# jonicho/simd-radix-sort

Measured on AMD Instinct MI355X. Metric: Gkeys/s and achieved HBM GB/s (% of roofline), 1e9 uint64 key+uint64 payload, higher is better.
Workload: dtype uint64; 1 GPU; c1: 1e9 uint64 keys + one uint64 payload column, uniform random; keys_per_gpu=1000000000, total_keys=1000000000, record_bytes=16, parallelism=1 GPU

## Files before the change

### include/srs_c_api.h

```cpp
#ifndef SRS_C_API_H_
#define SRS_C_API_H_

#include <stdint.h>

#ifdef __cplusplus
extern "C" {
#endif

typedef enum srs_key_kind {
  SRS_KEY_U8 = 0,
  SRS_KEY_I8 = 1,
  SRS_KEY_U16 = 2,
  SRS_KEY_I16 = 3,
  SRS_KEY_U32 = 4,
  SRS_KEY_I32 = 5,
  SRS_KEY_U64 = 6,
  SRS_KEY_I64 = 7,
  SRS_KEY_F32 = 8,
  SRS_KEY_F64 = 9
} srs_key_kind;

typedef enum srs_status {
  SRS_OK = 0,
  SRS_ERR_INVALID_ARG = -1,
// ... 62 lines not shown
                             const void* const* payloads, const uint32_t* payload_sizes,
                             void* keys_out, void* const* payloads_out,
                             int64_t* indices_out, void* stream);
int64_t srs_topk_rows_max_k(void);


int srs_key_histogram_device(int64_t num, int key_kind, int up, const void* keys,
                             int bits, uint64_t* hist, void* stream);

int srs_partition_device(int64_t num, int key_kind, int up, const void* keys,
                         int32_t num_payloads, const void* const* payloads,
                         const uint32_t* payload_sizes, int bits,
                         const int32_t* part_of_bucket, int32_t num_parts,
                         void* keys_out, void* const* payloads_out,
                         int64_t* part_counts, void* stream);

#define SRS_SHARD_ID_BYTES 128
typedef struct srs_shard_comm_s* srs_shard_comm;
int srs_shard_unique_id(void* id);
int srs_shard_comm_init(int32_t world, int32_t rank, const void* id, srs_shard_comm* comm);
int srs_shard_comm_init_all(int32_t num_devices, const int32_t* devices, srs_shard_comm* comms);
int srs_shard_comm_destroy(srs_shard_comm comm);

int srs_shard_comm_init_staged(int32_t world, srs_shard_comm* comms);

int srs_shard_set_options(srs_shard_comm comm, int32_t rounds, int32_t chunks);

int srs_shard_set_message_options(srs_shard_comm comm, int32_t self_messages,
                                  int64_t max_message_bytes);

int srs_shard_sort_device(srs_shard_comm comm, int64_t num, int key_kind, int up,
                          const void* keys, int32_t num_payloads, const void* const* payloads,
                          const uint32_t* payload_sizes, void** keys_out, void** payloads_out,
                          int64_t* num_out, void* stream);

int srs_shard_sort_multi(int32_t num_devices, const srs_shard_comm* comms, const int64_t* nums,
                         int key_kind, int up, const void* const* keys, int32_t num_payloads,
                         const void* const* payloads, const uint32_t* payload_sizes,
                         void** keys_out, void** payloads_out, int64_t* nums_out);

int srs_shard_last_report(srs_shard_comm comm, char* buf, int64_t cap);

int srs_shard_debug_inject(srs_shard_comm comm, int32_t point);

int srs_debug_shard_plan(int32_t world, int32_t rank, int32_t chunks, int32_t rounds,
                         int32_t key_bits, int32_t self_messages, const uint64_t* chunk_hists,
                         int64_t num, char* json, int64_t cap);


int srs_set_host_devices(int32_t num_devices, const int32_t* devices);


int srs_alloc_device(uint64_t bytes, void** ptr);
int srs_free_device(void* ptr);


int srs_fill_synthetic_device(int64_t num, int key_kind, uint64_t seed,
                              uint64_t first_index, void* keys,
                              int32_t num_payloads, void* const* payloads,
                              const uint32_t* payload_sizes, void* stream);


const char* srs_last_error(void);

const char* srs_version(void);

int srs_set_kernel_timing(int enable);
int srs_reset_kernel_stats(void);
int srs_kernel_stats(const char* name, int64_t* launches, double* total_ms,
                     double* elements);

int srs_debug_set_stamp_buffer(void* device_acc);

int srs_debug_set_lookback(void* status, void* err);

int srs_debug_set_super_scan(int64_t min_groups);

int srs_debug_last_fallbacks(int64_t* counts);

int srs_debug_last_local_counts(int64_t* counts);

int srs_debug_last_local_classes(int64_t* counts);

int srs_debug_alloc(uint64_t bytes, int mode, void** ptr);
int srs_debug_free(void* ptr);
int srs_debug_workspace(void** tmp, uint64_t* tmp_bytes, void** tmp2, uint64_t* tmp2_bytes);
int srs_debug_probe_write(void* ptr, uint64_t bytes, float* ms);

int srs_debug_plan_table(const uint32_t* hist, int64_t num, int key_bits, int32_t* mode,
                         int32_t* groups, double* overflow, double* overflow_other,
                         int32_t* table, int32_t* rbits);

int srs_release_workspace(void);

int srs_debug_set_topk_candidates(int64_t max_candidates);

int srs_debug_last_topk(int64_t* info);

int srs_debug_set_topk_rows_route(int route);

int srs_debug_last_topk_rows(int64_t* info);

#ifdef __cplusplus
}
#endif

#endif
```

### simd-radix-sort_amd/csrc/srs_api.hip

```cpp
#include <hip/hip_runtime.h>
#include <stdint.h>
#include <string.h>

#include <algorithm>
#include <atomic>
#include <chrono>
#include <cstring>
#include <cstdio>
#include <cstdlib>
#include <map>
#include <memory>
#include <mutex>
#include <queue>
#include <string>
#include <thread>
#include <vector>

#include "../../include/srs_c_api.h"
#include "srs_common.h"
#include "srs_kernels.h"

namespace srs {
namespace {

// ... 358 lines not shown
  auto it = g_pub_allocs.upper_bound(const_cast<void*>(p));
  if (it == g_pub_allocs.begin()) return false;
  --it;
  const char* a = (const char*)it->first;
  return (const char*)p >= a && (const char*)p + bytes <= a + it->second;
}

thread_local bool t_defer = false;
thread_local std::vector<std::pair<void*, int>> t_deferred;

hipError_t ws_free(void* p, int mode) {
  if (!p) return hipSuccess;
  if (t_defer) {
    t_deferred.push_back({p, mode});
    return hipSuccess;
  }
  return big_free(p, mode);
}

int ensure(DevBuf& b, size_t bytes, int mode = ALLOC_MALLOC, bool placed = false) {
  if (b.bytes >= bytes && b.p) return SRS_OK;
  if (b.p) {
    HIP_TRY(ws_free(b.p, b.mode));
    b.p = nullptr;
    b.bytes = 0;
  }
  size_t want = std::max<size_t>(bytes, 256);
  if (placed) HIP_TRY(placed_alloc(&b.p, want, mode));
  else HIP_TRY(big_alloc(&b.p, want, mode));
  b.bytes = want;
  b.mode = mode;
  return SRS_OK;
}

int ensure_keep(DevBuf& b, size_t bytes, size_t live_bytes, hipStream_t st) {
  if (b.bytes >= bytes && b.p) return SRS_OK;
  DevBuf nb;
  size_t want = std::max<size_t>(bytes, b.bytes * 2);
  HIP_TRY(hipMalloc(&nb.p, want));
  nb.bytes = want;
  if (b.p && live_bytes) HIP_TRY(hipMemcpyAsync(nb.p, b.p, live_bytes, hipMemcpyDeviceToDevice, st));
  if (b.p) {
    HIP_TRY(hipStreamSynchronize(st));
    HIP_TRY(ws_free(b.p, ALLOC_MALLOC));
  }
  b = nb;
  return SRS_OK;
}

inline void cpu_relax() {
#if defined(__x86_64__) || defined(__i386__)
  __builtin_ia32_pause();
#else
  std::this_thread::yield();
#endif
}

int sync_poll(hipStream_t st) {
  const auto t0 = std::chrono::steady_clock::now();
  for (;;) {
    const hipError_t q = hipStreamQuery(st);
    if (q == hipSuccess) return SRS_OK;
    if (q != hipErrorNotReady) HIP_TRY(q);
    const auto dt = std::chrono::steady_clock::now() - t0;
    if (dt > std::chrono::milliseconds(20)) break;
    if (dt < std::chrono::microseconds(200)) cpu_relax();
    else std::this_thread::yield();
  }
  HIP_TRY(hipStreamSynchronize(st));
  return SRS_OK;
}

struct Workspace {
  DevBuf tmp;
  DevBuf tmp2;
  DevBuf stage;
  DevBuf desc;
  DevBuf big[2], local, local2, copy, fallback, fallback2, redo, redo2;
  DevBuf plan, tcount, gcount, tbase, gbase, var, sbase;
  DevBuf tile_seg, group_seg, hist, offs, gsum, gofs, scan_tmp, totals, ctr;
  DevBuf shist, lut, lut_rbits;
  DevBuf prun, ptile, btot, bnt, btile, nt_over, gtile, gorder;
  int64_t gorder_cap = 0;
  DevBuf mid;
  DevBuf midbar;
  DevBuf sel, selhist, selcnt, seldesc;
  unsigned long long* h_sel = nullptr;
  int64_t topk_info[3] = {0, 0, 0};
  DevBuf rowspass;
  int64_t topk_rows_info[4] = {0, 0, 0, 0};
  bool rows_pass_pending = false;
  hipStream_t side = nullptr;
  hipEvent_t ev_fork = nullptr, ev_join = nullptr;
  ListCounters* h_ctr = nullptr;
  uint64_t* h_totals = nullptr;
  MidFlag* h_mid = nullptr;
  unsigned long long mid_seq = 0;
  hipEvent_t idle = nullptr;
  bool idle_pending = false;
  std::map<hipStream_t, DevBuf> small_taken;
  bool last_small = false;
  hipStream_t last_small_stream = nullptr;
  std::mutex mu;
  ~Workspace() {
    if (idle) {
      (void)hipEventSynchronize(idle);
      (void)hipEventDestroy(idle);
    }
    DevBuf* bufs[] = {&tmp, &tmp2, &stage, &desc, &big[0], &big[1], &local, &local2, &fallback,
                      &fallback2, &redo, &redo2, &shist, &lut, &lut_rbits, &copy, &plan, &tcount,
                      &gcount, &tbase, &gbase, &var, &sbase, &tile_seg, &group_seg, &hist, &offs,
                      &gsum, &gofs, &scan_tmp, &totals, &ctr, &prun, &ptile, &btot, &bnt, &btile,
                      &nt_over, &gtile, &gorder, &mid, &midbar, &sel, &selhist, &selcnt, &seldesc,
                      &rowspass};
    for (DevBuf* b : bufs) free_buf(*b);
    for (auto& t : small_taken) free_buf(t.second);
    if (h_sel) (void)hipHostFree(h_sel);
    if (h_ctr) (void)hipHostFree(h_ctr);
    if (h_totals) (void)hipHostFree(h_totals);
    if (h_mid) (void)hipHostFree(h_mid);
    if (side) (void)hipStreamDestroy(side);
    if (ev_fork) (void)hipEventDestroy(ev_fork);
    if (ev_join) (void)hipEventDestroy(ev_join);
    (void)hipGetLastError();
  }
};

std::mutex g_wmu;
std::map<int, std::shared_ptr<Workspace>>& g_ws = *new std::map<int, std::shared_ptr<Workspace>>;

struct WsLock {
  std::shared_ptr<Workspace> ref;
  std::unique_lock<std::mutex> lk;
};

int get_ws_locked(std::shared_ptr<Workspace>* out) {
  int dev = 0;
  HIP_TRY(hipGetDevice(&dev));
  auto it = g_ws.find(dev);
  if (it != g_ws.end()) {
    *out = it->second;
    return SRS_OK;
  }
  auto w = std::make_shared<Workspace>();
  HIP_TRY(hipHostMalloc((void**)&w->h_ctr, sizeof(ListCounters), hipHostMallocDefault));
  HIP_TRY(hipHostMalloc((void**)&w->h_totals, 4 * sizeof(uint64_t), hipHostMallocDefault));
  HIP_TRY(hipHostMalloc((void**)&w->h_mid, sizeof(MidFlag), hipHostMallocCoherent));
  memset(w->h_mid, 0, sizeof(MidFlag));
  g_ws[dev] = w;
  *out = w;
  return SRS_OK;
}

int acquire_ws(Workspace** out, WsLock* lk) {
  std::shared_ptr<Workspace> w;
  {
    std::lock_guard<std::mutex> g(g_wmu);
    SRS_TRY(get_ws_locked(&w));
  }
  lk->lk = std::unique_lock<std::mutex>(w->mu);
  lk->ref = std::move(w);
  *out = lk->ref.get();
  return SRS_OK;
}

size_t align_up(size_t x, size_t a) { return (x + a - 1) / a * a; }
// ... 447 lines not shown
      ok = (int)cl.size() <= kMaxRanges && cl.back().b1 - cl.back().b0 < kClusterSpan;
    }
    if (ok) {
      *clusters = cl;
      return SRS_OK;
    }
  }
  if (top9max * 512 <= (uint64_t)kBalancedSkew * total) {
    *spread = true;
    return SRS_OK;
  }
  if (R.aos) return SRS_OK;
  TablePlan P;
  plan_table(h, n, d.key_bits, &P);
  if (trace_levels() && P.mode)
    fprintf(stderr, "[srs] digit table mode %d: %d groups, predicted overflow %.0f keys (other "
            "table %.0f)\n", P.mode, P.groups, P.over, P.over_other);
  if (P.mode == 0) return SRS_OK;
  std::vector<int32_t>& rbits = P.rbits;
  if (P.mode == 3) {
    SRS_TRY(ensure(W->lut, 512 * sizeof(int32_t)));
    SRS_TRY(ensure(W->lut_rbits, kGroups * sizeof(int32_t)));
    HIP_TRY(hipMemcpyAsync(W->lut.p, P.tab3.data(), 512 * 4, hipMemcpyHostToDevice, st));
    HIP_TRY(hipMemcpyAsync(W->lut_rbits.p, rbits.data(), rbits.size() * 4, hipMemcpyHostToDevice,
                           st));
    HIP_TRY(hipStreamSynchronize(st));
    *lut_entries = 1024;
    *lut_mode = 3;
    *use = true;
    return SRS_OK;
  }
  const std::vector<int32_t>& lut = P.lut16;
  std::vector<uint16_t> t2(4096);
  for (int B = 0; B < 4096; B++) {
    bool same = true;
    for (int j = 1; j < 16; j++) same &= lut[B * 16 + j] == lut[B * 16];
    if (same) {
      t2[B] = (uint16_t)lut[B * 16];
    } else {
      const int idx = (int)(t2.size() - 4096) / 16;
      t2[B] = (uint16_t)(0x8000 | idx);
      for (int j = 0; j < 16; j++) t2.push_back((uint16_t)lut[B * 16 + j]);
    }
  }
  if ((int)t2.size() > kLdsLutEntries) return fail(SRS_ERR_INTERNAL, "digit table too large");
  *lut_entries = (int)t2.size();
  SRS_TRY(ensure(W->lut, align_up(t2.size() * sizeof(uint16_t), 16)));
  SRS_TRY(ensure(W->lut_rbits, kGroups * sizeof(int32_t)));
  HIP_TRY(hipMemcpyAsync(W->lut.p, t2.data(), t2.size() * 2, hipMemcpyHostToDevice, st));
  HIP_TRY(hipMemcpyAsync(W->lut_rbits.p, rbits.data(), rbits.size() * 4, hipMemcpyHostToDevice,
                         st));
  HIP_TRY(hipStreamSynchronize(st));
  *use = true;
  return SRS_OK;
}

int pair_tiles_mode(const SortDesc& d, int ks, bool aos_slices) {
  const char* e = getenv("SRS_PAIR_TILES");
  const int mode = e && *e ? atoi(e) : 2;
  if (mode == 0 || d.canon_zero || (ks != 4 && ks != 8)) return 0;
  const bool shape = d.cols[0].width == (uint32_t)ks &&
                     (d.pair ? ks == 4 && d.ncols == 3 : d.ncols <= 2);
  if (!shape) return 0;
  if (mode == 3) return 1 | 2;
  if (mode == 1) return 1;
  return aos_slices ? (1 | 4) : ks == 4 ? (1 | 2) : 1;
}

struct LevelState {
  int64_t nbig, n_local, n_local2, n_copy;
  int cur;
  int ncols;
  int tmp2;
  int64_t known_len = -1;
  int pair_tiles = 0;
  int level = 0;
};

struct LevelMode {
  int mode = 0;
  const GTile* gt = nullptr;
  const int32_t* nt_over = nullptr;
  const int32_t* torder = nullptr;
  int key_bits = 0;
  bool home = false;
};

int run_level(Workspace* W, int ks, const SortDesc* d_desc, LevelState& S, int force_bits,
              int lut, hipStream_t st, const int32_t* lut_rbits = nullptr,
              const LevelMode& M = LevelMode()) {
  const int64_t nbig = S.nbig;
  ListCounters* d_ctr = (ListCounters*)W->ctr.p;
  uint64_t* d_totals = (uint64_t*)W->totals.p;
  SRS_TRY(ensure(W->plan, nbig * sizeof(SegPlan)));
  SRS_TRY(ensure(W->tcount, nbig * 8));
  SRS_TRY(ensure(W->gcount, nbig * 8));
  SRS_TRY(ensure(W->tbase, nbig * 8));
  SRS_TRY(ensure(W->gbase, nbig * 8));
  SRS_TRY(ensure(W->var, nbig * 16));
  SRS_TRY(ensure(W->sbase, (size_t)nbig * kMaxBins * 8));
  SRS_TRY(ensure(W->scan_tmp, scan_temp_elems(nbig) * 8));
  SegPlan* plan = (SegPlan*)W->plan.p;
  unsigned long long* var = (unsigned long long*)W->var.p;
  const bool small_plan = nbig <= kPlanSmallMax;
  if (small_plan) {
    TimedScope ts("plan", (double)nbig, st);
    launch_plan_small((Seg*)W->big[S.cur].p, nbig, plan, (int64_t*)W->tbase.p,
                      (int64_t*)W->gbase.p, var, d_totals, &d_ctr->n_big, force_bits,
                      S.tmp2 | (M.home ? 2 : 0), st, M.nt_over);
  } else {
    TimedScope ts("plan", (double)nbig, st);
    HIP_TRY(hipMemsetAsync(d_totals + 3, 0, sizeof(uint64_t), st));
    launch_plan((Seg*)W->big[S.cur].p, nbig, plan, (int64_t*)W->tcount.p,
                (int64_t*)W->gcount.p, var, d_totals + 3, force_bits, S.tmp2 | (M.home ? 2 : 0),
                st, M.nt_over);
    launch_excl_scan((uint64_t*)W->tcount.p, (uint64_t*)W->tbase.p, nbig,
                     (uint64_t*)W->scan_tmp.p, d_totals + 0, st);
    launch_excl_scan((uint64_t*)W->gcount.p, (uint64_t*)W->gbase.p, nbig,
                     (uint64_t*)W->scan_tmp.p, d_totals + 1, st);
    launch_plan_bases(plan, nbig, (int64_t*)W->tbase.p, (int64_t*)W->gbase.p, st);
  }
  int64_t ntiles, ngroups;
  uint64_t level_keys;
  if (nbig == 1 && S.known_len >= 0) {
    level_keys = (uint64_t)S.known_len;
    ntiles = (S.known_len + kTile - 1) / kTile;
    ngroups = (ntiles + kScanGroup - 1) / kScanGroup;
  } else {
    HIP_TRY(hipMemcpyAsync(W->h_totals, d_totals, 4 * sizeof(uint64_t),
                           hipMemcpyDeviceToHost, st));
    SRS_TRY(sync_poll(st));
    ntiles = (int64_t)W->h_totals[0];
    ngroups = (int64_t)W->h_totals[1];
    level_keys = W->h_totals[3];
  }
  S.known_len = -1;
  const int lv = ++S.level;
  const double level_elems = (double)level_keys;
  note_elems("count", level_elems, lv);
  note_elems("scatter", level_elems, lv);

  SRS_TRY(ensure(W->tile_seg, ntiles * 4));
  SRS_TRY(ensure(W->group_seg, ngroups * 4));
  SRS_TRY(ensure(W->hist, (size_t)ntiles * kMaxBins * 2));
  const bool offs32 = level_keys < (1ull << 32);
  SRS_TRY(ensure(W->offs, (size_t)ntiles * kMaxBins * (offs32 ? 4 : 8)));
  const int64_t grows = ngroups + super_rows(ngroups);
  SRS_TRY(ensure(W->gsum, (size_t)grows * kMaxBins * 4));
  SRS_TRY(ensure(W->gofs, (size_t)grows * kMaxBins * 8));
  int32_t* tile_seg = (int32_t*)W->tile_seg.p;
  int32_t* group_seg = (int32_t*)W->group_seg.p;
  launch_seg_map2((int64_t*)W->tbase.p, ntiles, tile_seg, (int64_t*)W->gbase.p, ngroups,
                  group_seg, nbig, st);
  {
    TimedScope ts("count", (double)0, st, lv);
    launch_count(ks, d_desc, plan, tile_seg, ntiles, (uint16_t*)W->hist.p, var, var + nbig, lut, st,
                 M.gt, M.torder);
  }
  const size_t worst = (size_t)nbig * kMaxBins;
  const int nxt = S.cur ^ 1;
  SRS_TRY(ensure(W->big[nxt], worst * sizeof(Seg)));
  SRS_TRY(ensure_keep(W->local, (S.n_local + worst) * sizeof(Seg), S.n_local * sizeof(Seg), st));
  SRS_TRY(ensure_keep(W->local2, (S.n_local2 + worst) * sizeof(Seg), S.n_local2 * sizeof(Seg), st));
  SRS_TRY(ensure_keep(W->copy, (S.n_copy + worst) * sizeof(Seg), S.n_copy * sizeof(Seg), st));
  if (!small_plan)
    HIP_TRY(hipMemsetAsync(&d_ctr->n_big, 0, sizeof(unsigned long long), st));
  {
    TimedScope ts("scan", (double)ntiles, st);
    launch_offsets(plan, nbig, group_seg, ngroups, (uint16_t*)W->hist.p,
                   (uint32_t*)W->gsum.p, (uint64_t*)W->gofs.p, (uint64_t*)W->sbase.p,
                   offs32 ? nullptr : (uint64_t*)W->offs.p, offs32 ? (uint32_t*)W->offs.p : nullptr,
                   var, (Seg*)W->big[nxt].p, (Seg*)W->local.p,
                   (Seg*)W->local2.p, (Seg*)W->copy.p, d_ctr, lut_rbits, st, M.mode,
                   (uint32_t*)W->prun.p);
  }
  if (g_lb_status)
    HIP_TRY(hipMemsetAsync(g_lb_status, 0, (size_t)ntiles * kMaxBins * 4, st));
  {
    TimedScope ts("scatter", (double)0, st, lv);
    const bool pairs = (S.pair_tiles & 1) && (lut == 0 || ((S.pair_tiles & 2) && lut == 2)) &&
                       !((S.pair_tiles & 4) && lv == 1);
    if (pairs)
      launch_scatter_pairs(ks, d_desc, plan, tile_seg, (uint64_t*)W->offs.p,
                           offs32 ? (const uint32_t*)W->offs.p : nullptr, ntiles, lut, st, M.gt);
    else
      launch_scatter(ks, d_desc, plan, tile_seg, (uint64_t*)W->offs.p,
                     offs32 ? (const uint32_t*)W->offs.p : nullptr, ntiles, lut, S.ncols, st,
                     M.gt);
  }
  if (M.mode == 1) {
    const int nb = 1 << std::abs(force_bits);
    const int rbits = lut ? M.key_bits : M.key_bits - std::abs(force_bits);
    launch_stripe_tables((const uint32_t*)W->prun.p, nbig, nb, (uint32_t*)W->ptile.p,
                         (uint64_t*)W->btot.p, (uint32_t*)W->bnt.p, rbits, BUF_TMP,
                         (Seg*)W->big[nxt].p, (int32_t*)W->nt_over.p, (uint32_t*)W->btile.p,
                         d_ctr, (const uint64_t*)W->sbase.p, plan, (GTile*)W->gtile.p,
                         lut_rbits, st, (int32_t*)W->gorder.p, W->gorder_cap);
  }
  HIP_TRY(hipMemcpyAsync(W->h_ctr, d_ctr, sizeof(ListCounters), hipMemcpyDeviceToHost, st));
  SRS_TRY(sync_poll(st));
  S.nbig = (int64_t)W->h_ctr->n_big;
  S.n_local = (int64_t)W->h_ctr->n_local;
  S.n_local2 = (int64_t)W->h_ctr->n_local2;
  S.n_copy = (int64_t)W->h_ctr->n_copy;
  S.cur = nxt;
  if (trace_levels()) {
    fprintf(stderr, "[srs] level: %lld segs, %.0f keys, %lld tiles%s -> big %lld, local %lld, "
            "local2 %lld, copy %lld\n", (long long)nbig, level_elems, (long long)ntiles,
            lut ? " (lut)" : "", (long long)S.nbig, (long long)S.n_local,
            (long long)S.n_local2, (long long)S.n_copy);
    if (S.nbig > 0) {
      std::vector<Seg> b(S.nbig);
      HIP_TRY(hipMemcpy(b.data(), W->big[nxt].p, S.nbig * sizeof(Seg), hipMemcpyDeviceToHost));
      int64_t sum = 0, mx = 0, under16k = 0;
      for (const Seg& s : b) {
        sum += s.len;
        mx = std::max<int64_t>(mx, s.len);
        under16k += s.len <= 16384;
      }
      fprintf(stderr, "[srs]   big: %lld keys, max %lld, <= 16K keys: %lld segs; first rbits %d\n",
              (long long)sum, (long long)mx, (long long)under16k, b[0].rbits);
    }
  }
  return SRS_OK;
}

void set_columns(const Request& R, SortDesc& d, char* tmp, char* tmp2, bool aos_cols,
                 size_t slice_bytes, const size_t* tmp_off, bool inplace, bool pair = false) {
  const int ks = key_size_of(R.kind);
  if (R.aos) {
    const uint32_t E = R.elem_size;
    char* in = (char*)R.in_cols[0];
    char* out = (char*)R.out_cols[0];
    const uint32_t slice = E < 8 ? E : 8;
    int nc = 0;
    for (uint32_t off = 0; off < E; off += slice, nc++) {
      if (aos_cols)
        d.cols[nc] = Col{{in + off, out + off, tmp + nc * slice_bytes, tmp2 + nc * slice_bytes},
                         slice, {E, E, 8, 8}};
      else
        d.cols[nc] = Col{{in + off, out + off, tmp ? tmp + off : nullptr, nullptr}, slice,
                         {E, E, E, E}};
    }
    d.ncols = nc;
    d.key = d.cols[0];
    d.key.width = (uint32_t)ks;
  } else {
    for (int c = 0; c < R.ncols; c++) {
      const uint32_t w = R.widths[c];
      d.cols[c] = Col{{(char*)R.in_cols[c], (char*)R.out_cols[c], tmp ? tmp + tmp_off[c] : nullptr,
                       tmp2 ? tmp2 + tmp_off[c] : nullptr}, w, {w, w, w, w}};
    }
    if (pair) {
      for (int c = 1; c <= 2; c++) {
        const size_t off = tmp_off[1] + 4 * (c - 1);
        d.cols[c].base[BUF_TMP] = tmp + off;
        d.cols[c].base[BUF_TMP2] = tmp2 + off;
        d.cols[c].stride[BUF_TMP] = d.cols[c].stride[BUF_TMP2] = 8;
      }
      d.pair = 1;
    }
    d.key = d.cols[0];
    d.ncols = R.ncols;
  }
  if (inplace)
    for (int c = 0; c < d.ncols; c++) d.cols[c].base[BUF_IN] = d.cols[c].base[BUF_OUT];
}

bool is_inplace(const Request& R) {
  bool inplace = true;
  for (int c = 0; c < R.ncols; c++) inplace &= (R.in_cols[c] == R.out_cols[c]);
  return inplace;
}

int taken_slot(Workspace* W, hipStream_t st, DevBuf** out) {
  if (W->small_taken.size() >= 64 && !W->small_taken.count(st)) {
    HIP_TRY(hipDeviceSynchronize());
    for (auto& t : W->small_taken) free_buf(t.second);
    W->small_taken.clear();
    W->last_small = false;
  }
  DevBuf& taken = W->small_taken[st];
  SRS_TRY(ensure(taken, 2 * sizeof(int64_t)));
  *out = &taken;
  return SRS_OK;
}

int run_small(Workspace* W, const Request& R, hipStream_t st) {
  const int ks = key_size_of(R.kind);
  const int64_t n = R.num;
  const bool inplace = is_inplace(R);
  SortDesc d;
  memset(&d, 0, sizeof d);
  key_masks(R.kind, R.up, d);
  const bool is_float = R.kind == SRS_KEY_F32 || R.kind == SRS_KEY_F64;
  d.canon_zero = (is_float && n <= R.thresh) ? 1 : 0;
  d.leaf_skip = leaf_skip_of(R);
  const int ksl = ks | (d.canon_zero ? SRS_KS_CANON : 0);
  set_columns(R, d, nullptr, nullptr, false, 0, nullptr, inplace);
  d.stamp_acc = g_stamp_acc;
  const Seg g{0, n, d.key_bits, inplace ? BUF_OUT : BUF_IN};
  DevBuf* tk = nullptr;
  SRS_TRY(taken_slot(W, st, &tk));
  DevBuf& taken = *tk;
  W->last_small = true;
  W->last_small_stream = st;
  note_elems("local", (double)n);
  {
    TimedScope ts("local", (double)0, st);
    launch_small_sort(ksl, d, g, (int64_t*)taken.p, st);
  }
  HIP_TRY(hipGetLastError());
  return SRS_OK;
}

bool direct_layout_ok(const SortDesc& d, int pm, int ks) {
  const Col& k = d.cols[0];
  const int bufs[] = {BUF_IN, BUF_OUT, BUF_TMP, BUF_TMP2};
  if (pm == 0) {
    if (d.ncols != 2 || d.pair || d.cols[1].width != 8 || k.width != (uint32_t)ks) return false;
    for (int b : {BUF_IN, BUF_OUT, BUF_TMP, BUF_TMP2}) {
      if (b == BUF_TMP2 && !d.tmp2) continue;
      if (k.stride[b] != k.width || d.cols[1].stride[b] != 8) return false;
    }
    return true;
  }
  if (pm == 1) {
    const Col& p = d.cols[1];
    if (d.ncols != 2 || !d.tmp2 || ks != 8 || k.width != 8 || p.width != 8) return false;
    for (int b : {BUF_IN, BUF_OUT})
      if (k.stride[b] != 16 || p.stride[b] != 16 || p.base[b] != k.base[b] + 8) return false;
    for (int b : {BUF_TMP, BUF_TMP2})
      if (k.stride[b] != 8 || p.stride[b] != 8) return false;
    return true;
  }
  if (pm == 2) {
    const Col& a = d.cols[1];
    const Col& c = d.cols[2];
    if (d.ncols != 3 || !d.pair || a.width != 4 || c.width != 4 || k.width != (uint32_t)ks)
      return false;
    for (int b : bufs)
      if (k.stride[b] != k.width) return false;
    for (int b : {BUF_IN, BUF_OUT})
      if (a.stride[b] != 4 || c.stride[b] != 4) return false;
    for (int b : {BUF_TMP, BUF_TMP2})
      if (a.stride[b] != 8 || c.stride[b] != 8 || c.base[b] != a.base[b] + 4) return false;
    return true;
  }
  return false;
}

constexpr int64_t kStripeMinN = int64_t(1) << 25;

bool stripes_enabled() {
  static const bool on = [] {
    const char* e = getenv("SRS_NO_STRIPES");
    return !(e && *e && *e != '0');
  }();
  return on;
}

int plan_range_level(Workspace* W, const Request& R, const std::vector<KeyCluster>& cl,
                     SortDesc& d, hipStream_t st, bool* use, bool* final_lvl, bool* one_value) {
  *use = *final_lvl = *one_value = false;
  const int ks = key_size_of(R.kind);
  const int kb = 8 * ks;
  const int K = (int)cl.size();
  uint64_t hi[kMaxRanges] = {~0ull, ~0ull, ~0ull, ~0ull};
  for (int k = 0; k + 1 < K; k++) {
    const uint64_t mid_bin = ((uint64_t)cl[k].b1 + (uint64_t)cl[k + 1].b0 + 1) / 2;
    hi[k] = (mid_bin << (kb - 16)) - 1;
  }
  SRS_TRY(ensure(W->totals, 2 * kMaxRanges * sizeof(uint64_t)));
  unsigned long long* mm = (unsigned long long*)W->totals.p;
  uint64_t init[2 * kMaxRanges];
  for (int c = 0; c < kMaxRanges; c++) {
    init[2 * c] = ~0ull;
    init[2 * c + 1] = 0;
  }
  std::vector<uint64_t> got(2 * kMaxRanges);
  HIP_TRY(hipMemcpyAsync(mm, init, sizeof init, hipMemcpyHostToDevice, st));
  launch_key_minmax(R.in_cols[0], ks, ks, R.num, d.mpos, d.mneg, hi, mm, st);
  HIP_TRY(hipMemcpyAsync(got.data(), mm, sizeof init, hipMemcpyDeviceToHost, st));
  SRS_TRY(sync_poll(st));
  struct Rg {
    uint64_t mn, mx, cnt, hi;
  };
  std::vector<Rg> rg;
  for (int c = 0; c < K; c++) {
    if (got[2 * c] > got[2 * c + 1]) continue;
    rg.push_back(Rg{got[2 * c], got[2 * c + 1], std::max<uint64_t>(cl[c].cnt, 1), hi[c]});
  }
  if (rg.empty()) return SRS_OK;
  if (rg.size() == 1 && rg[0].mn == rg[0].mx) {
    *one_value = true;
    return SRS_OK;
  }
  const int R_ = (int)rg.size();
  auto shr = [](uint64_t x, int s) { return s >= 64 ? 0 : x >> s; };
  auto span = [&](int s) {
    uint64_t t = 0;
    for (const Rg& r : rg) t += shr(r.mx, s) - shr(r.mn, s) + 1;
    return t;
  };
  int s = 0;
  while (s < kb && span(s) > (uint64_t)kMaxBins) s++;
  uint32_t used = 0;
  for (int c = 0; c < kMaxRanges; c++) {
    d.rng_hi[c] = ~0ull;
    d.rng_adj[c] = 0;
  }
  std::vector<int> base(R_);
  for (int c = 0; c < R_; c++) {
    d.rng_hi[c] = c + 1 < R_ ? rg[c].hi : ~0ull;
    base[c] = (int)used;
    d.rng_adj[c] = used - (uint32_t)shr(rg[c].mn, s);
    used += (uint32_t)(shr(rg[c].mx, s) - shr(rg[c].mn, s) + 1);
  }
  std::vector<int32_t> rbits(kMaxBins, s);
  SRS_TRY(ensure(W->lut_rbits, kMaxBins * sizeof(int32_t)));
  HIP_TRY(hipMemcpyAsync(W->lut_rbits.p, rbits.data(), kMaxBins * sizeof(int32_t),
                         hipMemcpyHostToDevice, st));
  HIP_TRY(hipStreamSynchronize(st));
  d.digit_lut = nullptr;
  d.lut_mode = 2;
  d.lut_bits = kMaxDigitBits;
  d.lut_shift = s;
  d.lut_entries = 0;
  *use = true;
  *final_lvl = s == 0;
  if (trace_levels())
    for (int c = 0; c < R_; c++)
      fprintf(stderr, "[srs] range %d: keys [%llx, %llx] -> buckets from %d, shift %d\n", c,
              (unsigned long long)rg[c].mn, (unsigned long long)rg[c].mx, base[c], s);
  return SRS_OK;
}

int copy_through(const Request& R, hipStream_t st);

constexpr int64_t kHomeTmp2MinN = int64_t(1) << 24;

bool home_tmp2_enabled() {
  static const bool on = [] {
    const char* e = getenv("SRS_HOME_TMP2");
    return !(e && *e == '0');
  }();
  return on;
}

bool partition_pairs_enabled() {
  static const bool on = [] {
    const char* e = getenv("SRS_PARTITION_PAIRS");
    return !(e && *e == '0');
  }();
  return on;
}

constexpr int64_t kLocalForkMaxN = int64_t(1) << 24;
bool local_fork_enabled() {
  static const bool on = [] {
    const char* e = getenv("SRS_LOCAL_FORK");
    return !(e && *e == '0');
  }();
  return on;
}

bool mid_enabled() {
  static const bool on = [] {
    const char* e = getenv("SRS_MID");
    return !(e && *e == '0');
  }();
  return on;
}

int64_t mid_level_max_n() {
  static const int64_t v = [] {
    const char* e = getenv("SRS_MID_LEVEL_MAX");
    const int64_t x = e && *e ? (int64_t)atof(e) : kMidLevelMaxKeys;
    return std::min<int64_t>(x, kMidLevelMaxKeys);
  }();
  return v;
}

int wait_mid_flag(const MidFlag* f, unsigned long long seq, hipStream_t st) {
  auto seen = [&] { return __atomic_load_n(&f->seq, __ATOMIC_ACQUIRE) == seq; };
  const auto t0 = std::chrono::steady_clock::now();
  while (!seen()) {
    if (std::chrono::steady_clock::now() - t0 > std::chrono::milliseconds(5)) {
      HIP_TRY(hipStreamSynchronize(st));
      if (!seen()) return fail(SRS_ERR_INTERNAL, "mid-size launch: no answer from the kernel");
      break;
    }
    cpu_relax();
  }
  return SRS_OK;
}

int run_sort(Workspace* W, const Request& R, hipStream_t st) {
  if (R.nsegs == 0 && R.num <= kLocalCap) return run_small(W, R, st);
  {
    const char* e = getenv("SRS_XCD_ROT");
    set_xcd_rotation(e && *e ? atoi(e) : 0);
  }
  W->last_small = false;
  const int ks = key_size_of(R.kind);
  const int64_t n = R.num;
  const bool inplace = is_inplace(R);

  SortDesc d;
  memset(&d, 0, sizeof d);
  key_masks(R.kind, R.up, d);
  const bool is_float = R.kind == SRS_KEY_F32 || R.kind == SRS_KEY_F64;
  d.canon_zero = (is_float && n <= R.thresh) ? 1 : 0;
  d.leaf_skip = leaf_skip_of(R);
  const int ksl = ks | (d.canon_zero ? SRS_KS_CANON : 0);
  const bool mid = R.nsegs == 0 && n > kLocalCap && n <= kMidMaxKeys && mid_enabled();
  const bool mid1 = R.nsegs == 0 && n > kMidMaxKeys && n <= mid_level_max_n() && mid_enabled();

  const bool aos_cols = R.aos && R.elem_size >= 16 && n > kLocalCap && R.nsegs == 0 && !mid;
  const bool pair_cols = !R.aos && R.ncols == 3 && R.widths[1] == 4 && R.widths[2] == 4 &&
                         n > kLocalCap && R.nsegs == 0 && !mid && !mid1;
  bool home_tmp2 = false;
  if (!R.aos && !pair_cols && n >= kHomeTmp2MinN && R.nsegs == 0 && !mid && !mid1 &&
      home_tmp2_enabled()) {
    for (int c = 0; c < R.ncols && !home_tmp2; c++)
      home_tmp2 = !placed_memory(R.out_cols[c], (size_t)n * R.widths[c]);
  }
  size_t tmp_bytes = 0, slice_bytes = 0;
  std::vector<size_t> tmp_off;
  if (R.aos) {
    tmp_off.push_back(0);
    slice_bytes = align_up((size_t)n * 8, 256);
    tmp_bytes = aos_cols ? slice_bytes * (R.elem_size / 8) : align_up((size_t)n * R.elem_size, 256);
  } else {
    for (int c = 0; c < R.ncols; c++) {
      tmp_off.push_back(tmp_bytes);
      tmp_bytes += align_up((size_t)n * R.widths[c], 256);
    }
  }
  SRS_TRY(ensure(W->tmp, tmp_bytes, ws_alloc_mode(), true));
  char* tmp = (char*)W->tmp.p;
  char* tmp2 = nullptr;
  if (home_tmp2 && ensure(W->tmp2, tmp_bytes, ws_alloc_mode(), true) != SRS_OK) {
    home_tmp2 = false;
    (void)hipGetLastError();
  }
  if (aos_cols || pair_cols || home_tmp2) {
    SRS_TRY(ensure(W->tmp2, tmp_bytes, ws_alloc_mode(), true));
    tmp2 = (char*)W->tmp2.p;
    d.tmp2 = 1;
  }

  set_columns(R, d, tmp, tmp2, aos_cols, slice_bytes, tmp_off.data(), inplace, pair_cols);

  d.stamp_acc = g_stamp_acc;
  d.lb_status = g_lb_status;
  d.lb_err = g_lb_err;
  bool balanced = false, spread = false, ranges = false, ranges_final = false;
  int lut_entries = 0, lut_mode = 1;
  std::vector<KeyCluster> clusters;
  SRS_TRY(plan_balanced_level(W, R, d, &balanced, &lut_entries, &lut_mode, st, &spread,
                              &clusters));
  if (!clusters.empty()) {
    bool one_value = false;
    SRS_TRY(plan_range_level(W, R, clusters, d, st, &ranges, &ranges_final, &one_value));
    if (one_value) return copy_through(R, st);
    balanced = ranges;
  }
  if (balanced && !ranges) {
    d.digit_lut = (const int32_t*)W->lut.p;
    d.lut_shift = d.key_bits - (lut_mode == 3 ? 9 : 16);
    d.lut_bits = lut_mode == 3 ? 9 : 16;
    d.lut_mode = lut_mode;
    d.lut_entries = lut_entries;
  }
  SRS_TRY(ensure(W->desc, sizeof(SortDesc)));
  SortDesc* d_desc = (SortDesc*)W->desc.p;

  const int home = inplace ? BUF_OUT : BUF_IN;
  SRS_TRY(ensure(W->big[0], 1024 * sizeof(Seg)));
  SRS_TRY(ensure(W->big[1], 1024 * sizeof(Seg)));
  SRS_TRY(ensure(W->local, 1024 * sizeof(Seg)));
  SRS_TRY(ensure(W->local2, 1024 * sizeof(Seg)));
  SRS_TRY(ensure(W->copy, 1024 * sizeof(Seg)));
  SRS_TRY(ensure(W->ctr, sizeof(ListCounters)));
  SRS_TRY(ensure(W->totals, 4 * sizeof(uint64_t)));
  ListCounters* d_ctr = (ListCounters*)W->ctr.p;
// ... 86 lines not shown
          W->last_small_stream = st;
          return SRS_OK;
        }
        launch_set_desc(d, d_desc, st);
        W->h_ctr->local_elems = 0;
        started = true;
      }
    }
    if (mid1) {
      const int64_t T = (n + kTile - 1) / kTile;
      const int64_t part_bytes = mid_level_part_bytes();
      SRS_TRY(ensure(W->mid, part_bytes + T * kMaxBins * sizeof(uint32_t)));
      if (!W->midbar.p) {
        SRS_TRY(ensure(W->midbar, mid_bar_words() * sizeof(unsigned long long)));
        HIP_TRY(hipMemsetAsync(W->midbar.p, 0, mid_bar_words() * sizeof(unsigned long long), st));
      }
      auto barrier_failed = [&] { return __atomic_load_n(&W->h_mid->err, __ATOMIC_ACQUIRE) != 0; };
      if (barrier_failed())
        return fail(SRS_ERR_INTERNAL, "mid-size launch: a grid barrier timed out");
      hipError_t e;
      const unsigned long long seq = ++W->mid_seq;
      {
        note_elems("mid_level", (double)n);
        TimedScope ts("mid_level", (double)0, st);
        e = launch_mid_level(ksl, d, n, home, (unsigned long long*)W->mid.p,
                             (uint32_t*)((char*)W->mid.p + part_bytes), d_ctr, (Seg*)W->big[0].p,
                             (Seg*)W->local.p, (Seg*)W->local2.p, (Seg*)W->copy.p, d_desc,
                             W->h_mid, seq, (unsigned long long*)W->midbar.p, st);
      }
      if (e != hipSuccess) {
        (void)hipGetLastError();
        if (trace_levels())
          fprintf(stderr, "[srs] mid-level launch refused (%s): general path\n", hipGetErrorString(e));
      } else {
        SRS_TRY(wait_mid_flag(W->h_mid, seq, st));
        if (barrier_failed())
          return fail(SRS_ERR_INTERNAL, "mid-size launch: a grid barrier timed out");
        n_big = (int64_t)__atomic_load_n(&W->h_mid->n_big, __ATOMIC_ACQUIRE);
        n_local = (int64_t)__atomic_load_n(&W->h_mid->n_local, __ATOMIC_ACQUIRE);
        n_local2 = (int64_t)__atomic_load_n(&W->h_mid->n_local2, __ATOMIC_ACQUIRE);
        n_copy = (int64_t)__atomic_load_n(&W->h_mid->n_copy, __ATOMIC_ACQUIRE);
        W->h_ctr->local_elems = __atomic_load_n(&W->h_mid->local_elems, __ATOMIC_ACQUIRE);
        if (trace_levels())
          fprintf(stderr, "[srs] mid-level: big %lld, local %lld, local2 %lld, copy %lld\n",
                  (long long)n_big, (long long)n_local, (long long)n_local2, (long long)n_copy);
        if (n_big + n_local + n_local2 + n_copy == 0) return SRS_OK;
        started = true;
      }
    }
    if (!started) {
      Seg seg0{0, n, d.key_bits, home};
      const bool to_local = n <= kLocalCap;
      launch_start(d, d_desc, seg0, to_local ? 1 : 0, (Seg*)W->big[0].p, (Seg*)W->local.p,
                   (Seg*)W->local2.p, d_ctr, st);
      n_big = to_local ? 0 : 1;
      n_local = (to_local && n <= kLocalCapSmall) ? 1 : 0;
      n_local2 = (to_local && n > kLocalCapSmall) ? 1 : 0;
      W->h_ctr->local_elems = to_local ? (uint64_t)n : 0;
    } else {
      mid_continued = true;
    }
  }
  LevelState S{n_big, n_local, n_local2, n_copy, 0, d.ncols, d.tmp2};
  S.pair_tiles = pair_tiles_mode(d, ks, aos_cols);
  if (R.nsegs == 0 && n_big == 1 && !mid_continued) S.known_len = n;
  if (one_seg_len > 0) S.known_len = one_seg_len;
  int level = 0;
  const int b1 = balanced ? kMaxDigitBits : choose_bits(n, d.key_bits);
  const int64_t stripe_len = (int64_t)kStripeKeysPerBucket << b1;
  const bool stripes = R.nsegs == 0 && !d.canon_zero && (ks == 4 || ks == 8) &&
                       (balanced || spread) && !ranges_final &&
                       n >= kStripeMinN && n < (int64_t(1) << 32) && n >= 2 * stripe_len &&
                       stripes_enabled();
  if (stripes) {
    const int64_t K = (n + stripe_len - 1) / stripe_len;
    std::vector<Seg> hs(K);
    for (int64_t k = 0; k < K; k++)
      hs[k] = Seg{k * stripe_len, std::min(stripe_len, n - k * stripe_len), d.key_bits, home};
    SRS_TRY(ensure(W->big[0], K * sizeof(Seg)));
    HIP_TRY(hipMemcpyAsync(W->big[0].p, hs.data(), K * sizeof(Seg), hipMemcpyHostToDevice, st));
    const int nb = 1 << b1;
    const size_t pieces = (size_t)K * kMaxBins;
    SRS_TRY(ensure(W->prun, pieces * 4));
    SRS_TRY(ensure(W->ptile, pieces * 4));
    SRS_TRY(ensure(W->btot, kMaxBins * 8));
    SRS_TRY(ensure(W->bnt, kMaxBins * 4));
    SRS_TRY(ensure(W->btile, kMaxBins * 4));
    SRS_TRY(ensure(W->nt_over, kMaxBins * 4));
    SRS_TRY(ensure(W->gtile, ((n + kTile - 1) / kTile + (size_t)K * nb) * sizeof(GTile)));
    W->gorder_cap = (n + kTile - 1) / kTile + (int64_t)K * nb;
    SRS_TRY(ensure(W->gorder, (W->gorder_cap + K) * sizeof(int32_t)));
    HIP_TRY(hipStreamSynchronize(st));
    S.nbig = K;
    S.known_len = -1;
    LevelMode m1;
    m1.mode = 1;
    m1.key_bits = d.key_bits;
    ++level;
    if (balanced)
      SRS_TRY(run_level(W, ksl, d_desc, S, kMaxDigitBits, d.lut_mode >= 2 ? 2 : 1, st,
                        (const int32_t*)W->lut_rbits.p, m1));
    else
      SRS_TRY(run_level(W, ksl, d_desc, S, -b1, false, st, nullptr, m1));
    LevelMode m2;
    m2.mode = 2;
    m2.gt = (const GTile*)W->gtile.p;
    m2.nt_over = (const int32_t*)W->nt_over.p;
    m2.torder = (const int32_t*)W->gorder.p;
    ++level;
    if (S.nbig > 0) SRS_TRY(run_level(W, ksl, d_desc, S, 0, false, st, nullptr, m2));
  }
  if (balanced && !stripes && S.nbig > 0) {
    ++level;
    LevelMode m0;
    m0.home = ranges_final;
    SRS_TRY(run_level(W, ksl, d_desc, S, kMaxDigitBits, d.lut_mode >= 2 ? 2 : 1, st,
                      (const int32_t*)W->lut_rbits.p, m0));
  }
  while (S.nbig > 0) {
    if (++level > 80) return fail(SRS_ERR_INTERNAL, "level limit exceeded");
    SRS_TRY(run_level(W, ksl, d_desc, S, 0, false, st));
  }
  n_local = S.n_local;
  n_local2 = S.n_local2;
  n_copy = S.n_copy;

  if (n_local + n_local2 > 0) {
    note_elems("local", (double)W->h_ctr->local_elems);
    TimedScope ts("local", (double)0, st);
    SRS_TRY(ensure(W->fallback, (n_local + n_local2) * sizeof(Seg)));
    SRS_TRY(ensure(W->fallback2, (n_local + n_local2) * sizeof(Seg)));
    Seg* fb = (Seg*)W->fallback.p;
    Seg* fb1 = fb + n_local2;
    Seg* fb2 = (Seg*)W->fallback2.p;
    unsigned long long* nfb = &d_ctr->n_fallback;
    unsigned long long* nfb1 = &d_ctr->n_fallback1;
    unsigned long long* nfb2 = &d_ctr->n_fallback2;
    hipStream_t s2 = st;
    if (n_local > 0 && n_local2 > 0 && n <= kLocalForkMaxN && local_fork_enabled()) {
      if (!W->side) {
        HIP_TRY(hipStreamCreateWithFlags(&W->side, hipStreamNonBlocking));
        HIP_TRY(hipEventCreateWithFlags(&W->ev_fork, hipEventDisableTiming));
        HIP_TRY(hipEventCreateWithFlags(&W->ev_join, hipEventDisableTiming));
      }
      HIP_TRY(hipEventRecord(W->ev_fork, st));
      HIP_TRY(hipStreamWaitEvent(W->side, W->ev_fork, 0));
      s2 = W->side;
    }
    {
      TimedScope ts1("local_fast", 0, st);
      const bool rec16 = aos_cols && R.elem_size == 16;
      int pm = -1;
      if (!R.aos && R.ncols == 2 && R.widths[1] == 8 && !d.pair) pm = 0;
      else if (rec16 && ks == 8) pm = 1;
      else if (d.pair && ks == 4) pm = 2;
      if (pm >= 0 && !direct_layout_ok(d, pm, ks)) pm = -1;
      const bool direct_any = pm >= 0 && (ks == 4 || ks == 8) && !d.canon_zero &&
                              direct_local_enabled();
      const bool direct = direct_any && n_local >= direct_min_segs();
      const bool direct2 = direct_any && direct_local2_enabled() && n_local2 >= direct_min_segs();
      if (n_local2 > 0 && direct2) {
        SRS_TRY(ensure(W->redo2, n_local2 * sizeof(Seg)));
        launch_local_direct(ks, pm, d_desc, (Seg*)W->local2.p, n_local2, (Seg*)W->redo2.p,
                            &d_ctr->n_redo2, fb, nfb, s2, true);
        launch_local_list(ks, d_desc, (Seg*)W->redo2.p, &d_ctr->n_redo2,
                          (int)std::min<int64_t>(n_local2, 1024), fb, nfb, s2, true);
      } else if (n_local2 > 0) {
        launch_local(ksl, d_desc, (Seg*)W->local2.p, n_local2, 1, fb, nfb, s2, rec16);
      }
      if (n_local > 0 && direct) {
        SRS_TRY(ensure(W->redo, n_local * sizeof(Seg)));
        launch_local_direct(ks, pm, d_desc, (Seg*)W->local.p, n_local, (Seg*)W->redo.p,
                            &d_ctr->n_redo, fb1, nfb1, st);
        launch_local_list(ks, d_desc, (Seg*)W->redo.p, &d_ctr->n_redo,
                          (int)std::min<int64_t>(n_local, 2048), fb1, nfb1, st);
      } else if (n_local > 0) {
        launch_local(ksl, d_desc, (Seg*)W->local.p, n_local, 0, fb1, nfb1, st, rec16);
      }
    }
    {
// ... 1308 lines not shown
int srs_set_host_devices(int32_t num_devices, const int32_t* devices) {
  if (num_devices < 0 || num_devices > 512 || (num_devices > 0 && !devices))
    return fail(SRS_ERR_INVALID_ARG, "num_devices must be in [0, 512] with a device array");
  int ndev = 0;
  if (num_devices > 0 && (hipGetDeviceCount(&ndev) != hipSuccess || ndev == 0))
    return fail(SRS_ERR_NO_DEVICE, "no HIP device available");
  for (int i = 0; i < num_devices; i++)
    if (devices[i] < 0 || devices[i] >= ndev)
      return fail(SRS_ERR_INVALID_ARG, "no such device in the host device list");
  std::lock_guard<std::mutex> g(g_hdmu);
  g_host_devs.assign(devices, devices + num_devices);
  g_host_devs_set = true;
  return SRS_OK;
}

int srs_set_kernel_timing(int enable) {
  std::lock_guard<std::mutex> lk(g_tmu);
  g_timing = enable == 2 ? 2 : enable != 0;
  return SRS_OK;
}

int srs_reset_kernel_stats(void) {
  std::lock_guard<std::mutex> lk(g_tmu);
  drain_timing_locked();
  g_stats.clear();
  return SRS_OK;
}

int srs_kernel_stats(const char* name, int64_t* launches, double* total_ms, double* elements) {
  std::lock_guard<std::mutex> lk(g_tmu);
  drain_timing_locked();
  if (!name) return fail(SRS_ERR_INVALID_ARG, "name is NULL");
  auto it = g_stats.find(name);
  const KStat k = it == g_stats.end() ? KStat{} : it->second;
  if (launches) *launches = k.launches;
  if (total_ms) *total_ms = k.ms;
  if (elements) *elements = k.elems;
  return SRS_OK;
}

int srs_debug_set_stamp_buffer(void* device_acc) {
  g_stamp_acc = (unsigned long long*)device_acc;
  return SRS_OK;
}

int srs_debug_set_lookback(void* status, void* err) {
  g_lb_status = (uint32_t*)status;
  g_lb_err = (unsigned long long*)err;
  return SRS_OK;
}

int srs_debug_last_local_counts(int64_t* counts) {
  if (!counts) return fail(SRS_ERR_INVALID_ARG, "counts is NULL");
  Workspace* W = nullptr;
  WsLock lk;
  SRS_TRY(acquire_ws(&W, &lk));
  counts[0] = counts[1] = 0;
  if (W->last_small || !W->ctr.p) return SRS_OK;
  HIP_TRY(hipDeviceSynchronize());
  ListCounters c;
  HIP_TRY(hipMemcpy(&c, W->ctr.p, sizeof c, hipMemcpyDeviceToHost));
  counts[0] = (int64_t)(c.n_local + c.n_local2);
  counts[1] = (int64_t)(c.n_redo + c.n_redo2);
  return SRS_OK;
}

int srs_debug_last_local_classes(int64_t* counts) {
  if (!counts) return fail(SRS_ERR_INVALID_ARG, "counts is NULL");
  Workspace* W = nullptr;
  WsLock lk;
  SRS_TRY(acquire_ws(&W, &lk));
  counts[0] = counts[1] = counts[2] = counts[3] = 0;
  if (W->last_small || !W->ctr.p) return SRS_OK;
  HIP_TRY(hipDeviceSynchronize());
  ListCounters c;
  HIP_TRY(hipMemcpy(&c, W->ctr.p, sizeof c, hipMemcpyDeviceToHost));
  counts[0] = (int64_t)c.n_local;
  counts[1] = (int64_t)c.n_local2;
  counts[2] = (int64_t)c.n_redo;
  counts[3] = (int64_t)c.n_redo2;
  return SRS_OK;
}

int srs_debug_set_super_scan(int64_t min_groups) {
  set_super_scan_min_groups(min_groups);
  return SRS_OK;
}

int srs_debug_last_fallbacks(int64_t* counts) {
  if (!counts) return fail(SRS_ERR_INVALID_ARG, "counts is NULL");
  Workspace* W = nullptr;
  WsLock lk;
  SRS_TRY(acquire_ws(&W, &lk));
  counts[0] = counts[1] = 0;
  if (W->last_small) {
    HIP_TRY(hipDeviceSynchronize());
    HIP_TRY(hipMemcpy(counts, W->small_taken[W->last_small_stream].p, 2 * sizeof(int64_t),
                      hipMemcpyDeviceToHost));
    return SRS_OK;
  }
  if (!W->ctr.p) return SRS_OK;
  HIP_TRY(hipDeviceSynchronize());
  ListCounters c;
  HIP_TRY(hipMemcpy(&c, W->ctr.p, sizeof c, hipMemcpyDeviceToHost));
  counts[0] = (int64_t)(c.n_fallback + c.n_fallback1);
  counts[1] = (int64_t)c.n_fallback2;
  return SRS_OK;
}

int srs_debug_plan_table(const uint32_t* hist, int64_t num, int key_bits, int32_t* mode,
                         int32_t* groups, double* overflow, double* overflow_other,
                         int32_t* table, int32_t* rbits) {
  if (!hist || !mode || !table || !rbits || (key_bits != 32 && key_bits != 64) || num < 1)
    return fail(SRS_ERR_INVALID_ARG, "srs_debug_plan_table: arguments");
  std::vector<uint32_t> h(hist, hist + 65536);
  TablePlan P;
  plan_table(h, num, key_bits, &P);
  *mode = P.mode;
  if (groups) *groups = P.groups;
  if (overflow) *overflow = P.over;
  if (overflow_other) *overflow_other = P.over_other;
  if (P.mode == 1) memcpy(table, P.lut16.data(), 65536 * 4);
  if (P.mode == 3) memcpy(table, P.tab3.data(), 512 * 4);
  if (P.mode) memcpy(rbits, P.rbits.data(), kGroups * 4);
  return SRS_OK;
}

int srs_alloc_device(uint64_t bytes, void** ptr) {
  if (!ptr) return fail(SRS_ERR_INVALID_ARG, "srs_alloc_device: ptr is NULL");
  *ptr = nullptr;
  if (bytes == 0) return SRS_OK;
  HIP_TRY(placed_alloc(ptr, (size_t)bytes, ALLOC_MALLOC));
  std::lock_guard<std::mutex> g(g_pub_amu);
  g_pub_allocs[*ptr] = (size_t)bytes;
  return SRS_OK;
}

int srs_free_device(void* ptr) {
  if (!ptr) return SRS_OK;
  {
    std::lock_guard<std::mutex> g(g_pub_amu);
    auto it = g_pub_allocs.find(ptr);
    if (it == g_pub_allocs.end())
      return fail(SRS_ERR_INVALID_ARG, "srs_free_device: not from srs_alloc_device");
    g_pub_allocs.erase(it);
  }
  HIP_TRY(hipFree(ptr));
  return SRS_OK;
}

std::mutex g_dbg_amu;
std::map<void*, int> g_dbg_allocs;

int srs_debug_alloc(uint64_t bytes, int mode, void** ptr) {
  if (!ptr || mode < ALLOC_MALLOC || mode >= ALLOC_MODES || bytes == 0)
    return fail(SRS_ERR_INVALID_ARG, "srs_debug_alloc: ptr, mode 0..4 and bytes > 0");
  HIP_TRY(big_alloc(ptr, (size_t)bytes, mode));
  std::lock_guard<std::mutex> g(g_dbg_amu);
  g_dbg_allocs[*ptr] = mode;
  return SRS_OK;
}

int srs_debug_free(void* ptr) {
  int mode = 0;
  {
    std::lock_guard<std::mutex> g(g_dbg_amu);
// ... 91 lines not shown
```

### simd-radix-sort_amd/csrc/srs_common.h

```cpp
#pragma once

#include <hip/hip_runtime.h>
#include <stdint.h>

namespace srs {

enum BufId : int32_t { BUF_IN = 0, BUF_OUT = 1, BUF_TMP = 2, BUF_TMP2 = 3 };
constexpr int kNumBufs = 4;

struct Col {
  char* base[kNumBufs];
  uint32_t width;
  uint32_t stride[kNumBufs];
};

#define SRS_MAX_COLS 65

struct SortDesc {
  Col key;
  Col cols[SRS_MAX_COLS];
  int32_t ncols;
  int32_t key_bits;
  int32_t canon_zero;
  int32_t tmp2;
  int32_t pair;
  int32_t leaf_skip;
  uint64_t mpos, mneg, signbit, negzero;
  const int32_t* digit_lut;
  int32_t lut_shift;
  int32_t lut_bits;
  int32_t lut_mode;
  int32_t lut_entries;
  uint64_t rng_hi[4];
  uint32_t rng_adj[4];
  unsigned long long* stamp_acc;
  uint32_t* lb_status;
  unsigned long long* lb_err;
};

struct Seg {
  int64_t start;
  int64_t len;
  int32_t rbits;
  int32_t buf;
};

struct SegPlan {
  int64_t start;
  int64_t len;
  int64_t tile_base;
  int64_t group_base;
  int32_t ntiles;
  int32_t ngroups;
  int32_t shift;
  int32_t bits;
  int32_t buf;
  int32_t dst;
  int32_t skip;
};

struct GTile {
  int64_t src;
  int32_t cnt;
  int32_t pad;
};
#ifndef SRS_STRIPE_KPB
#define SRS_STRIPE_KPB 3904
#endif
constexpr int kStripeKeysPerBucket = SRS_STRIPE_KPB;

struct MidFlag {
  unsigned long long n_big;
  unsigned long long seq;
  unsigned long long err;
  unsigned long long n_local, n_local2, n_copy, local_elems;
};

struct ListCounters {
  unsigned long long n_big;
  unsigned long long n_local;
  unsigned long long n_copy;
  unsigned long long local_elems;
  unsigned long long n_local2;
  unsigned long long n_fallback;
  unsigned long long n_fallback1;
  unsigned long long n_fallback2;
  unsigned long long n_redo;
  unsigned long long n_redo2;
};

#ifndef SRS_SCATTER_THREADS
#define SRS_SCATTER_THREADS 1024
#endif
#ifndef SRS_SCATTER_ITEMS
#define SRS_SCATTER_ITEMS 4
#endif
#ifndef SRS_SCATTER_WAVES_PER_EU
#define SRS_SCATTER_WAVES_PER_EU 8
#endif
#ifndef SRS_SCATTER_SDIG
#define SRS_SCATTER_SDIG 1
#endif
#ifndef SRS_LOCAL_RANK_SPLIT
#define SRS_LOCAL_RANK_SPLIT 2
#endif
constexpr int kScatterThreads = SRS_SCATTER_THREADS;
constexpr int kScatterItems = SRS_SCATTER_ITEMS;
constexpr int kTile = kScatterThreads * kScatterItems;
#ifndef SRS_COUNT_THREADS
#define SRS_COUNT_THREADS 256
#endif
constexpr int kCountThreads = SRS_COUNT_THREADS;
constexpr int kCountItems = kTile / kCountThreads;
static_assert(kCountItems * kCountThreads == kTile, "count block shape");
#ifndef SRS_MAX_DIGIT_BITS
#define SRS_MAX_DIGIT_BITS 9
#endif
constexpr int kMaxDigitBits = SRS_MAX_DIGIT_BITS;
#define SRS_KS_CANON 0x100
constexpr int kMaxBins = 1 << kMaxDigitBits;
static_assert(kScatterThreads >= kMaxBins, "the scatter tile scan gives one bin per thread");
#ifndef SRS_SCAN_GROUP
#define SRS_SCAN_GROUP 32
#endif
constexpr int kScanGroup = SRS_SCAN_GROUP;
constexpr int kHistMaxBits = 12;
constexpr int kMaxRanges = 4;
constexpr int kLdsLutBits = 12;
constexpr int kLdsLutEntries = 4096 + 16 * 512;
constexpr int kSampleWGs = 256;
constexpr int kSampleChunk = 1024;
constexpr int kSampleMaxChunks = 4096;
static_assert((kSampleMaxChunks + kSampleWGs - 1) / kSampleWGs * kSampleChunk < 65536,
              "sample histogram: u16 bins per workgroup");

#ifndef SRS_LOCAL_THREADS
#define SRS_LOCAL_THREADS 1024
#endif
#ifndef SRS_LOCAL_ITEMS
#define SRS_LOCAL_ITEMS 8
#endif
constexpr int kLocalItems = SRS_LOCAL_ITEMS;
constexpr int kLocalThreads = SRS_LOCAL_THREADS;
constexpr int kLocalCap = kLocalThreads * kLocalItems;
#ifndef SRS_LOCAL_SMALL_THREADS
#define SRS_LOCAL_SMALL_THREADS 512
#endif
// ... 74 lines not shown
```

### simd-radix-sort_amd/csrc/srs_kernels.h

```cpp
#pragma once

#include <hip/hip_runtime.h>
#include <stdint.h>

#include "srs_common.h"

namespace srs {

void launch_plan(const Seg* big, int64_t nbig, SegPlan* plan, int64_t* tcount,
                 int64_t* gcount, unsigned long long* var_or, uint64_t* elems, int force_bits,
                 int tmp2, hipStream_t st, const int32_t* nt_over = nullptr);
void launch_plan_small(const Seg* big, int64_t nbig, SegPlan* plan, int64_t* tbase,
                       int64_t* gbase, unsigned long long* var_or, uint64_t* totals,
                       unsigned long long* n_big_next, int force_bits, int tmp2,
                       hipStream_t st, const int32_t* nt_over = nullptr);
constexpr int64_t kPlanSmallMax = 16384;
void launch_seg_map2(const int64_t* tbase, int64_t ntiles, int32_t* tile_seg,
                     const int64_t* gbase, int64_t ngroups, int32_t* group_seg, int64_t nbig,
                     hipStream_t st);
void launch_start(const SortDesc& d, SortDesc* out, Seg seg0, int to_local, Seg* big, Seg* local,
                  Seg* local2, ListCounters* ctr, hipStream_t st);
void launch_plan_bases(SegPlan* plan, int64_t nbig, const int64_t* tbase,
                       const int64_t* gbase, hipStream_t st);
void launch_count(int key_size, const SortDesc* d, const SegPlan* plan,
                  const int32_t* tile_seg, int64_t ntiles, uint16_t* hist,
                  unsigned long long* var_or, unsigned long long* var_and, int lut,
                  hipStream_t st, const GTile* gt = nullptr, const int32_t* torder = nullptr);
int64_t scan_temp_elems(int64_t n);
void launch_excl_scan(const uint64_t* x, uint64_t* y, int64_t n, uint64_t* temp,
                      uint64_t* total, hipStream_t st);
int64_t super_rows(int64_t ngroups);
void set_super_scan_min_groups(int64_t g);
void launch_offsets(SegPlan* plan, int64_t nbig, const int32_t* group_seg, int64_t ngroups,
                    const uint16_t* hist, uint32_t* gsum, uint64_t* gofs, uint64_t* sbase,
                    uint64_t* offs, uint32_t* offs32, const unsigned long long* var_or,
                    Seg* big_next, Seg* local, Seg* local2, Seg* copy, ListCounters* ctr,
                    const int32_t* lut_rbits, hipStream_t st, int mode = 0,
                    uint32_t* prun = nullptr);
void launch_scatter(int key_size, const SortDesc* d, const SegPlan* plan,
                    const int32_t* tile_seg, const uint64_t* offs, const uint32_t* offs32,
                    int64_t ntiles, int lut, int ncols, hipStream_t st,
                    const GTile* gt = nullptr);
void launch_scatter_pairs(int key_size, const SortDesc* d, const SegPlan* plan,
                          const int32_t* tile_seg, const uint64_t* offs, const uint32_t* offs32,
                          int64_t ntiles, int lut, hipStream_t st, const GTile* gt = nullptr);
void launch_stripe_tables(const uint32_t* prun, int64_t nstripes, int nb, uint32_t* ptile,
                          uint64_t* btot, uint32_t* bnt, int rbits, int buf, Seg* big,
                          int32_t* nt_over, uint32_t* btile, ListCounters* ctr,
                          const uint64_t* sbase, const SegPlan* plan, GTile* gt,
                          const int32_t* lut_rbits, hipStream_t st, int32_t* torder = nullptr,
                          int64_t tiles_cap = 0);
void launch_key_hist(int key_size, int64_t n, const void* keys, const SortDesc& d, int bits,
                     unsigned long long* hist, hipStream_t st);
void launch_local(int key_size, const SortDesc* d, const Seg* segs, int64_t nsegs, int big_class,
                  Seg* fallback, unsigned long long* fallback_count, hipStream_t st,
                  bool rec16 = false);
void launch_local_direct(int key_size, int pm, const SortDesc* d, const Seg* segs, int64_t nsegs,
                         Seg* redo, unsigned long long* redo_count, Seg* fallback,
                         unsigned long long* fallback_count, hipStream_t st, bool big = false);
void launch_local_list(int key_size, const SortDesc* d, const Seg* segs,
                       const unsigned long long* nsegs, int grid, Seg* fallback,
                       unsigned long long* fallback_count, hipStream_t st, bool big = false);
void launch_local_stable(int key_size, const SortDesc* d, const Seg* segs,
                         const unsigned long long* nsegs, int big_class, Seg* fallback,
                         unsigned long long* fallback_count, int grid, hipStream_t st);
void launch_small_sort(int key_size, const SortDesc& d, Seg g, int64_t* taken, hipStream_t st);
constexpr int kMidMaxKeys = 256 * kTile;
int mid_bar_words();
int64_t mid_part_bytes(int64_t n);
hipError_t launch_mid_sort(int key_size, const SortDesc& d, int64_t n, int src,
                           unsigned long long* part, uint32_t* hist, ListCounters* ctr, Seg* big,
                           unsigned long long* taken, MidFlag* flag, unsigned long long seq,
                           unsigned long long* bar, hipStream_t st);
constexpr int kMidLevelMaxKeys = 1024 * kTile;
int64_t mid_level_part_bytes();
hipError_t launch_mid_level(int key_size, const SortDesc& d, int64_t n, int src,
                            unsigned long long* part, uint32_t* hist, ListCounters* ctr, Seg* big,
                            Seg* local, Seg* local2, Seg* copy, SortDesc* d_out, MidFlag* flag,
                            unsigned long long seq, unsigned long long* bar, hipStream_t st);
void launch_local_lsd(int key_size, const SortDesc* d, const Seg* segs,
                      const unsigned long long* nsegs, int grid, hipStream_t st);
int64_t sample_partial_bytes();
void launch_key_minmax(const void* keys, int key_bytes, int elem_bytes, int64_t n, uint64_t mpos,
                       uint64_t mneg, const uint64_t* hi, unsigned long long* mm, hipStream_t st);
bool launch_sample_hist16(const void* keys, int key_bytes, int elem_bytes, int64_t n,
                          int64_t stride, int chunk, int64_t blocks, uint64_t mpos, uint64_t mneg,
                          uint32_t* partial, uint32_t* hist, hipStream_t st);
void launch_fill(int64_t n, int kind, uint64_t seed, uint64_t first, void* keys,
                 int npay, const Col* pays, hipStream_t st);
void launch_set_desc(const SortDesc& d, SortDesc* out, hipStream_t st);
float probe_write_ms(void* buf, size_t bytes, hipStream_t st);
void set_xcd_rotation(int mode);
void launch_copy_list(const SortDesc* d, const Seg* segs, int64_t nsegs, uint64_t* chunks,
                      uint64_t* cbase, uint64_t* scan_temp, uint64_t* total, hipStream_t st);


struct SelectArgs {
  const char* keys;
  uint32_t stride;
  int32_t all;
  int64_t n;
  uint64_t pv;
  int32_t psh;
  int32_t shift, bits;
  int32_t key_bits;
  uint64_t mpos, mneg;
};
constexpr int kSelOrSlot = 1 << kHistMaxBits;
constexpr int kSelHistWords = kSelOrSlot + 2;
void launch_select_hist(int key_size, const SelectArgs& a, unsigned long long* hist,
                        hipStream_t st);
void launch_select_tally(int key_size, const SelectArgs& a, uint64_t* counts, hipStream_t st);
void launch_select_gather(int key_size, const SelectArgs& a, const SortDesc* d,
                          const uint64_t* tbase, int64_t limit, int64_t* idx_out, hipStream_t st);

struct TopkRowsCol {
  const char* in;
  char* out;
  uint32_t width;
};
struct TopkRowsArgs {
  int64_t rows, row_len, row_stride, kk;
  int32_t ncols;
  int32_t key_bits;
  uint64_t mpos, mneg;
  int32_t cap;
  int32_t select;
  int64_t* idx_out;
  unsigned long long* max_passes;
  TopkRowsCol col[SRS_MAX_COLS];
};
constexpr int kTopkRowsMaxK = 2048;
constexpr int kTopkRowsStreamCap = 2 * kTopkRowsMaxK;
constexpr int kTopkRowsMinCap = 256;
// ... 5 lines not shown
```

### simd-radix-sort_amd/csrc/srs_kernels.hip

```cpp
#include <hip/hip_runtime.h>
#include <stdint.h>

#include <algorithm>
#include <atomic>
#include <type_traits>

#include "srs_common.h"
#include "srs_kernels.h"

namespace srs {

#define SRS_GLOBAL __attribute__((address_space(1)))
template <typename T>
__device__ __forceinline__ T gld(const void* p) {
  return *(const SRS_GLOBAL T*)(p);
}
template <typename T>
__device__ __forceinline__ void gst(void* p, T v) {
#if SRS_DIAG_NT_STORES
  __builtin_nontemporal_store(v, (SRS_GLOBAL T*)(p));
#else
  *(SRS_GLOBAL T*)(p) = v;
#endif
}
// ... 12 lines not shown
  if constexpr (W == 1) return gld<uint8_t>(p);
  else if constexpr (W == 2) return gld<uint16_t>(p);
  else if constexpr (W == 4) return gld<uint32_t>(p);
  else return gld<uint64_t>(p);
}

template <int W>
__device__ __forceinline__ void stw(char* p, uint64_t v) {
  if constexpr (W == 1) gst<uint8_t>(p, (uint8_t)v);
  else if constexpr (W == 2) gst<uint16_t>(p, (uint16_t)v);
  else if constexpr (W == 4) gst<uint32_t>(p, (uint32_t)v);
  else gst<uint64_t>(p, v);
}

template <int W>
struct WidthTag {
  static constexpr int value = W;
};

template <typename F>
__device__ __forceinline__ void with_width(uint32_t w, F&& f) {
  switch (w) {
    case 1: f(WidthTag<1>{}); break;
    case 2: f(WidthTag<2>{}); break;
    case 4: f(WidthTag<4>{}); break;
    default: f(WidthTag<8>{}); break;
  }
}

__device__ __forceinline__ void store_w(char* p, uint32_t w, uint64_t v) {
  switch (w) {
    case 1: gst<uint8_t>(p, (uint8_t)v); break;
    case 2: gst<uint16_t>(p, (uint16_t)v); break;
    case 4: gst<uint32_t>(p, (uint32_t)v); break;
    default: gst<uint64_t>(p, v); break;
  }
}

template <int IT, bool DENSE = false, int FW = 0, typename F>
__device__ __forceinline__ void with_strip(uint32_t w, uint32_t st, F&& f) {
  if constexpr (FW != 0) {
    static_assert(DENSE, "fixed width implies a dense strip here");
    f(WidthTag<FW>{}, std::integral_constant<bool, true>{});
  } else if (DENSE || st == w) {
    with_width(w, [&](auto W_) { f(W_, std::integral_constant<bool, true>{}); });
  } else {
    with_width(w, [&](auto W_) { f(W_, std::integral_constant<bool, false>{}); });
  }
}

__device__ __forceinline__ __amdgpu_buffer_rsrc_t strip_rsrc(const char* base, uint32_t bytes) {
  const uint64_t b = (uint64_t)base;
  const uint32_t lo = __builtin_amdgcn_readfirstlane((uint32_t)b);
  const uint32_t hi = __builtin_amdgcn_readfirstlane((uint32_t)(b >> 32));
  const uint32_t n = __builtin_amdgcn_readfirstlane(bytes);
  return __builtin_amdgcn_make_buffer_rsrc((void*)(((uint64_t)hi << 32) | lo), (short)0, (int)n,
                                           0x00020000);
}

template <int W, int AUX = 0>
__device__ __forceinline__ uint64_t bld(__amdgpu_buffer_rsrc_t r, uint32_t voff, uint32_t soff = 0) {
  if constexpr (W == 1) return __builtin_amdgcn_raw_buffer_load_b8(r, voff, soff, AUX);
  else if constexpr (W == 2) return __builtin_amdgcn_raw_buffer_load_b16(r, voff, soff, AUX);
  else if constexpr (W == 4) return __builtin_amdgcn_raw_buffer_load_b32(r, voff, soff, AUX);
  else {
    const auto v = __builtin_amdgcn_raw_buffer_load_b64(r, voff, soff, AUX);
    return (uint64_t)v[0] | ((uint64_t)v[1] << 32);
  }
}

template <int IT, bool DENSE = false, int FW = 0, int AUX = 0>
__device__ __forceinline__ void load_strip(uint64_t (&dst)[IT], const char* src, uint32_t w,
                                           uint32_t st, int64_t first, int ebase, int cnt) {
  const __amdgpu_buffer_rsrc_t r =
      strip_rsrc(src + first * (int64_t)st, cnt > 0 ? (uint32_t)cnt * st : 0u);
  with_strip<IT, DENSE, FW>(w, st, [&](auto W_, auto D_) {
    constexpr int W = decltype(W_)::value;
    constexpr bool D = decltype(D_)::value;
    const uint32_t o0 = (uint32_t)ebase * (D ? (uint32_t)W : st);
#pragma unroll
    for (int k = 0; k < IT; k++) {
      if constexpr (D) dst[k] = bld<W, AUX>(r, o0 + (uint32_t)k * 64u * W);
      else dst[k] = bld<W, AUX>(r, o0, __builtin_amdgcn_readfirstlane((uint32_t)k * 64u * st));
    }
  });
}

template <int W>
__device__ __forceinline__ void bst(__amdgpu_buffer_rsrc_t r, uint64_t v, uint32_t voff,
                                    uint32_t soff = 0) {
  if constexpr (W == 1) __builtin_amdgcn_raw_buffer_store_b8((uint8_t)v, r, voff, soff, 0);
  else if constexpr (W == 2) __builtin_amdgcn_raw_buffer_store_b16((uint16_t)v, r, voff, soff, 0);
  else if constexpr (W == 4) __builtin_amdgcn_raw_buffer_store_b32((uint32_t)v, r, voff, soff, 0);
  else {
    typedef uint32_t u32x2 __attribute__((ext_vector_type(2)));
    u32x2 x;
    x[0] = (uint32_t)v;
    x[1] = (uint32_t)(v >> 32);
    __builtin_amdgcn_raw_buffer_store_b64(x, r, voff, soff, 0);
  }
}

template <int IT, bool DENSE = false, int FW = 0, typename V>
__device__ __forceinline__ void store_strip(char* out, uint32_t w, uint32_t st, int64_t first,
                                            int ebase, int cnt, V&& value) {
  const __amdgpu_buffer_rsrc_t r =
      strip_rsrc(out + first * (int64_t)st, cnt > 0 ? (uint32_t)cnt * st : 0u);
  with_strip<IT, DENSE, FW>(w, st, [&](auto W_, auto D_) {
    constexpr int W = decltype(W_)::value;
    constexpr bool D = decltype(D_)::value;
    const uint32_t o0 = (uint32_t)ebase * (D ? (uint32_t)W : st);
#pragma unroll
    for (int k = 0; k < IT; k++) {
      if constexpr (D) bst<W>(r, value(k), o0 + (uint32_t)k * 64u * W);
      else bst<W>(r, value(k), o0, __builtin_amdgcn_readfirstlane((uint32_t)k * 64u * st));
    }
  });
}

template <typename U, bool CZ = false>
struct Xform {
  U mpos, cdiff, negzero;
  int sbit;
  bool canon;
  __device__ __forceinline__ void init(const SortDesc& d) {
    mpos = (U)d.mpos;
    cdiff = (U)(d.mpos ^ d.mneg);
    negzero = (U)d.negzero;
    sbit = d.key_bits - 1;
    canon = d.canon_zero != 0;
  }
  __device__ __forceinline__ U operator()(U bits) const {
    if constexpr (CZ) {
      if (canon && bits == negzero) bits = 0;
    }
    U sm;
    if constexpr (sizeof(U) == 8) sm = (U)((int64_t)bits >> 63);
    else sm = (U)__builtin_amdgcn_sbfe((int)bits, sbit, 1);
    return bits ^ mpos ^ (sm & cdiff);
  }
  __device__ __forceinline__ U inv(U u) const {
    const U x = u ^ mpos;
    U sm;
    if constexpr (sizeof(U) == 8) sm = (U)((int64_t)x >> 63);
    else sm = (U)__builtin_amdgcn_sbfe((int)x, sbit, 1);
    return x ^ (sm & cdiff);
  }
};

__device__ __forceinline__ uint32_t lane_id() { return threadIdx.x & 63; }

struct DigitLut {
  const uint16_t* s;
  const int32_t* g;
  int shift;
  int mode;
  const SortDesc* r;
};

template <int LUT, typename U>
__device__ __forceinline__ uint32_t pass_digit(U u, int shift, uint32_t mask, const DigitLut& L) {
  if constexpr (LUT) {
    if (L.mode == 2) {
      const uint64_t v = (uint64_t)u;
      const SortDesc* d = L.r;
      const uint32_t a = v > d->rng_hi[2] ? d->rng_adj[3]
// ... 348 lines not shown
  else if (m == 4) l = (local + xcd * len / 16) % len;
  return start + l;
}

template <int LUT>
constexpr int kLutLdsEntries = LUT == 1 ? kLdsLutEntries : LUT == 2 ? 1024 : 8;

template <int LUT, int NT>
__device__ __forceinline__ DigitLut stage_lut(const SortDesc* desc, uint16_t* slut) {
  DigitLut L{};
  if (!LUT) return L;
  L.shift = desc->lut_shift;
  L.mode = desc->lut_mode;
  L.r = desc;
  if constexpr (LUT == 2) {
    if (L.mode == 3) {
      typedef uint32_t u32x4 __attribute__((ext_vector_type(4)));
      const __amdgpu_buffer_rsrc_t r = strip_rsrc((const char*)desc->digit_lut, 2048u);
      for (uint32_t i = threadIdx.x; i < 128u; i += NT)
        ((u32x4*)slut)[i] = __builtin_amdgcn_raw_buffer_load_b128(r, i * 16u, 0, 0);
      L.s = slut;
    }
    return L;
  }
  if (L.mode == 2) {
  } else if (L.mode == 3) {
    typedef uint32_t u32x4 __attribute__((ext_vector_type(4)));
    const __amdgpu_buffer_rsrc_t r = strip_rsrc((const char*)desc->digit_lut, 2048u);
    for (uint32_t i = threadIdx.x; i < 128u; i += NT)
      ((u32x4*)slut)[i] = __builtin_amdgcn_raw_buffer_load_b128(r, i * 16u, 0, 0);
    L.s = slut;
  } else if (L.mode == 1) {
    const int n8 = (desc->lut_entries + 7) >> 3;
    constexpr int K = (kLdsLutEntries / 8 + NT - 1) / NT;
    const __amdgpu_buffer_rsrc_t r = strip_rsrc((const char*)desc->digit_lut, (uint32_t)n8 * 16u);
    typedef uint32_t u32x4 __attribute__((ext_vector_type(4)));
    u32x4 v[K];
#pragma unroll
    for (int k = 0; k < K; k++)
      v[k] = __builtin_amdgcn_raw_buffer_load_b128(r, (threadIdx.x + (uint32_t)k * NT) * 16u, 0, 0);
#pragma unroll
    for (int k = 0; k < K; k++) {
      const int i = threadIdx.x + k * NT;
      if (i < n8) ((u32x4*)slut)[i] = v[k];
    }
    L.s = slut;
  } else if (desc->lut_bits < 2) {
    for (int i = threadIdx.x; i < (1 << desc->lut_bits); i += NT)
      slut[i] = (uint16_t)gld<int32_t>(desc->digit_lut + i);
    L.s = slut;
  } else if (desc->lut_bits <= kLdsLutBits) {
    const int n4 = (1 << desc->lut_bits) >> 2;
    constexpr int K = ((1 << kLdsLutBits) / 4 + NT - 1) / NT;
    const __amdgpu_buffer_rsrc_t r = strip_rsrc((const char*)desc->digit_lut, (uint32_t)n4 * 16u);
    typedef uint32_t u32x4 __attribute__((ext_vector_type(4)));
    u32x4 v[K];
#pragma unroll
    for (int k = 0; k < K; k++)
      v[k] = __builtin_amdgcn_raw_buffer_load_b128(r, (threadIdx.x + (uint32_t)k * NT) * 16u, 0, 0);
#pragma unroll
    for (int k = 0; k < K; k++) {
      const int i = threadIdx.x + k * NT;
      if (i < n4) {
        ((uint32_t*)slut)[2 * i] = (v[k][0] & 0xFFFFu) | (v[k][1] << 16);
        ((uint32_t*)slut)[2 * i + 1] = (v[k][2] & 0xFFFFu) | (v[k][3] << 16);
      }
    }
    L.s = slut;
  } else {
    L.g = desc->digit_lut;
  }
  return L;
}

#ifndef SRS_COUNT_TILES
#define SRS_COUNT_TILES 1
#endif
constexpr int kCountTiles = SRS_COUNT_TILES;

struct CountTile {
  int64_t t;
  int32_t s;
  int32_t cnt;
  bool vec;
};

template <typename KT>
__device__ __forceinline__ int count_elem(bool vec, int k) {
  constexpr int KB = (int)sizeof(KT);
  constexpr int PER = KB >= 4 ? 16 / KB : 1;
  return vec ? ((k / PER) * kCountThreads + (int)threadIdx.x) * PER + k % PER
             : k * kCountThreads + (int)threadIdx.x;
}

template <typename KT, typename U>
__device__ __forceinline__ CountTile count_load(const SortDesc* __restrict__ desc,
                                                const SegPlan* __restrict__ plan,
                                                const int32_t* __restrict__ tile_seg,
                                                const GTile* __restrict__ gt, int64_t t,
                                                int64_t ntiles, U (&raw)[kCountItems]) {
  CountTile T;
  T.t = t;
  T.cnt = 0;
  T.s = 0;
  T.vec = false;
  if (t >= ntiles) {
#pragma unroll
    for (int k = 0; k < kCountItems; k++) raw[k] = 0;
    return T;
  }
  T.s = tile_seg[t];
  const SegPlan P = plan[T.s];
  const char* kp = desc->key.base[P.buf];
  const uint32_t ks = desc->key.stride[P.buf];
  int64_t base;
  if (gt) {
    base = gt[t].src;
    T.cnt = gt[t].cnt;
  } else {
    const int64_t tl = t - P.tile_base;
    base = P.start + tl * kTile;
    const int64_t rem = P.len - tl * kTile;
    T.cnt = rem < kTile ? (int)rem : kTile;
  }
  constexpr int KB = (int)sizeof(KT);
  constexpr int PER = KB >= 4 ? 16 / KB : 1;
  static_assert(kCountItems % PER == 0, "whole 16-byte pieces per thread");
  T.vec = KB >= 4 && ks == (uint32_t)KB;
  const int cnt = T.cnt;
  if (T.vec) {
    typedef uint32_t u32x4 __attribute__((ext_vector_type(4)));
    const __amdgpu_buffer_rsrc_t r =
        strip_rsrc(kp + base * (int64_t)KB, cnt > 0 ? (uint32_t)cnt * KB : 0u);
    u32x4 c[kCountItems / PER];
#pragma unroll
    for (int j = 0; j < kCountItems / PER; j++)
      c[j] = __builtin_amdgcn_raw_buffer_load_b128(
          r, (threadIdx.x + (uint32_t)j * kCountThreads) * 16u, 0, 0);
#pragma unroll
    for (int k = 0; k < kCountItems; k++) {
      const u32x4 v = c[k / PER];
      if constexpr (KB == 8)
        raw[k] = (U)((uint64_t)v[2 * (k % PER)] | ((uint64_t)v[2 * (k % PER) + 1] << 32));
      else
        raw[k] = (U)v[k % PER];
    }
  } else {
#pragma unroll
    for (int k = 0; k < kCountItems; k++) {
      const int e = count_elem<KT>(false, k);
      raw[k] = e < cnt ? (U)gld<KT>(kp + (base + e) * (int64_t)ks) : (U)0;
    }
  }
  return T;
}

template <typename KT, typename U, int LUT, bool CZ>
__device__ __forceinline__ void count_add(const SortDesc* __restrict__ desc,
                                          const SegPlan* __restrict__ plan, const CountTile& T,
                                          const U (&raw)[kCountItems],
                                          uint32_t* h, unsigned long long* sor,
                                          const DigitLut& lut) {
  if (T.cnt == 0) return;
  const SegPlan P = plan[T.s];
  const uint32_t mask = (1u << P.bits) - 1;
  Xform<U, CZ> xf;
  xf.init(*desc);
  const int cnt = T.cnt;
  U vor = 0, vand = ~(U)0;
  bool agg;
  {
    const uint32_t d = pass_digit<LUT>(xf(raw[0]), P.shift, mask, lut);
    const uint32_t d0 = __builtin_amdgcn_readfirstlane(d);
    const bool ok0 = count_elem<KT>(T.vec, 0) < cnt;
    agg = __ballot(ok0 && d == d0) == __ballot(ok0);
  }
  const bool full = cnt == kTile;
  auto digit_of = [&](int k, bool& ok) -> uint32_t {
    ok = full || count_elem<KT>(T.vec, k) < cnt;
    const U u = xf(raw[k]);
    vor |= ok ? u : (U)0;
    vand &= ok ? u : ~(U)0;
    return ok ? pass_digit<LUT>(u, P.shift, mask, lut) : (uint32_t)kMaxBins;
  };
  if (!agg) {
#pragma unroll
    for (int k = 0; k < kCountItems; k++) {
      bool ok;
      atomicAdd(&h[digit_of(k, ok)], 1u);
    }
  } else {
#pragma unroll
    for (int k = 0; k < kCountItems; k++) {
      bool ok;
      const uint32_t d = digit_of(k, ok);
      const uint32_t d0 = __builtin_amdgcn_readfirstlane(d);
      const uint64_t vm = __ballot(ok);
      if (__ballot(d != d0) == 0) {
        if (lane_id() == 0) atomicAdd(&h[d0], (uint32_t)__popcll(vm));
      } else {
        atomicAdd(&h[d], 1u);
      }
    }
  }
#pragma unroll
  for (int o = 32; o >= 1; o >>= 1) {
    vor |= __shfl_xor(vor, o, 64);
    vand &= __shfl_xor(vand, o, 64);
  }
  if (lane_id() == 0) {
    atomicOr(&sor[0], (unsigned long long)vor);
    atomicAnd(&sor[1], (unsigned long long)vand);
  }
}

__device__ __forceinline__ void count_flush(const SegPlan* __restrict__ plan, const CountTile& T,
                                            uint32_t* h, unsigned long long* sor,
                                            uint16_t* __restrict__ hist,
                                            unsigned long long* __restrict__ var_or,
                                            unsigned long long* __restrict__ var_and) {
  static_assert(kTile < 65536, "u16 tile counts");
  if (T.cnt == 0) return;
  const uint32_t nb = 1u << plan[T.s].bits;
  uint32_t* row = (uint32_t*)(hist + T.t * kMaxBins);
  for (uint32_t i = threadIdx.x; i < nb / 2; i += kCountThreads) {
    row[i] = h[2 * i] | (h[2 * i + 1] << 16);
    h[2 * i] = 0;
    h[2 * i + 1] = 0;
  }
  if (threadIdx.x == 0) {
    const unsigned long long o = sor[0], a = sor[1];
    sor[0] = 0;
    sor[1] = ~0ull;
    const unsigned long long ko =
// ... 217 lines not shown
        run += a[k];
      }
    }
    for (; g + 4 <= g1; g += 4) {
      const uint32_t a0 = gsum[(g + 0) * kMaxBins + b], a1 = gsum[(g + 1) * kMaxBins + b];
      const uint32_t a2 = gsum[(g + 2) * kMaxBins + b], a3 = gsum[(g + 3) * kMaxBins + b];
      gofs[(g + 0) * kMaxBins + b] = run;
      gofs[(g + 1) * kMaxBins + b] = run + a0;
      gofs[(g + 2) * kMaxBins + b] = run + a0 + a1;
      gofs[(g + 3) * kMaxBins + b] = run + a0 + a1 + a2;
      run += (uint64_t)a0 + a1 + a2 + a3;
    }
    for (; g < g1; g++) {
      gofs[g * kMaxBins + b] = run;
      run += gsum[g * kMaxBins + b];
    }
  }
  uint64_t tot;
  const uint64_t ex = block_excl_scan<kMaxBins>(run, scan_sh, &tot);
  if (b < nb) sbase[s * kMaxBins + b] = ex;
  if (b < nb && (int64_t)run == P.len && mode == 0) single = 1;
  if (mode == 1) {
    if (b < nb) prun[s * kMaxBins + b] = (uint32_t)run;
    return;
  }
  __syncthreads();
  Seg c;
  c.len = 0;
  if (single) {
    if (b == 0) {
      plan[s].skip = 1;
      const unsigned long long v = var_or[s] ^ var_or[gridDim.x + s];
      c.start = P.start;
      c.len = P.len;
      c.rbits = v ? 64 - __clzll((long long)v) : 0;
      if (c.rbits > P.shift) c.rbits = P.shift;
      c.buf = P.buf;
    }
  } else if (b < nb && run > 0) {
    c.start = P.start + (int64_t)ex;
    c.len = (int64_t)run;
    c.rbits = (lut_rbits && lut_rbits[b] < P.shift) ? lut_rbits[b] : P.shift;
    c.buf = P.dst;
  }
  emit_children_block(Lists{big_next, local, local2, copy, ctr}, c);
}

__global__ __launch_bounds__(kMaxBins) void tile_offs_kernel(
    const SegPlan* __restrict__ plan, const int32_t* __restrict__ group_seg,
    const uint16_t* __restrict__ hist, const uint64_t* __restrict__ gofs,
    const uint64_t* __restrict__ sbase, uint64_t* __restrict__ offs,
    uint32_t* __restrict__ offs32) {
  const int64_t g = blockIdx.x;
  const int32_t s = group_seg[g];
  const SegPlan P = plan[s];
  const uint32_t b = threadIdx.x;
  if (P.skip || b >= (1u << P.bits)) return;
  const int64_t t0 = P.tile_base + (g - P.group_base) * kScanGroup;
  const int64_t t1 = min(t0 + kScanGroup, P.tile_base + P.ntiles);
  uint64_t run = sbase[s * kMaxBins + b] + gofs[g * kMaxBins + b];
  auto body = [&](auto* out) {
    using O = std::remove_pointer_t<decltype(out)>;
    int64_t t = t0;
    for (; t + 4 <= t1; t += 4) {
      const uint32_t a0 = hist[(t + 0) * kMaxBins + b], a1 = hist[(t + 1) * kMaxBins + b];
      const uint32_t a2 = hist[(t + 2) * kMaxBins + b], a3 = hist[(t + 3) * kMaxBins + b];
      out[(t + 0) * kMaxBins + b] = (O)run;
      out[(t + 1) * kMaxBins + b] = (O)(run + a0);
      out[(t + 2) * kMaxBins + b] = (O)(run + a0 + a1);
      out[(t + 3) * kMaxBins + b] = (O)(run + a0 + a1 + a2);
      run += (uint64_t)a0 + a1 + a2 + a3;
    }
    for (; t < t1; t++) {
      const uint32_t a = hist[t * kMaxBins + b];
      out[t * kMaxBins + b] = (O)run;
      run += a;
    }
  };
  if (offs32) body(offs32);
  else body(offs);
}

constexpr int kStripeThreads = 256;
__global__ __launch_bounds__(kStripeThreads) void stripe_tiles_kernel(
    const uint32_t* __restrict__ prun, int64_t nstripes, uint32_t* __restrict__ ptile,
    uint64_t* __restrict__ btot, uint32_t* __restrict__ bnt) {
  __shared__ uint64_t sh[kStripeThreads / 64 + 1];
  __shared__ uint64_t sh2[kStripeThreads / 64 + 1];
  const int b = blockIdx.x;
  uint64_t tiles = 0, keys = 0;
  for (int64_t s0 = 0; s0 < nstripes; s0 += kStripeThreads) {
    const int64_t s = s0 + threadIdx.x;
    const uint32_t len = s < nstripes ? prun[s * kMaxBins + b] : 0u;
    const uint64_t nt = (len + kTile - 1) / kTile;
    uint64_t tt, kt;
    const uint64_t ex = block_excl_scan<kStripeThreads>(nt, sh, &tt);
    block_excl_scan<kStripeThreads>((uint64_t)len, sh2, &kt);
    if (s < nstripes) ptile[s * kMaxBins + b] = (uint32_t)(tiles + ex);
    tiles += tt;
    keys += kt;
  }
  if (threadIdx.x == 0) {
    btot[b] = keys;
    bnt[b] = (uint32_t)tiles;
  }
}

__global__ __launch_bounds__(kMaxBins) void stripe_segs_kernel(
    const uint64_t* __restrict__ btot, const uint32_t* __restrict__ bnt, int nb, int rbits,
    int buf, Seg* __restrict__ big, int32_t* __restrict__ nt_over,
    uint32_t* __restrict__ btile, ListCounters* __restrict__ ctr,
    const int32_t* __restrict__ lut_rbits) {
  __shared__ uint64_t sh[3][kMaxBins / 64 + 1];
  const int b = threadIdx.x;
  const uint64_t len = b < nb ? btot[b] : 0;
  const uint64_t nt = b < nb ? bnt[b] : 0;
  const uint64_t used = len > 0 ? 1 : 0;
  uint64_t tot_len, tot_nt, tot_used;
  const uint64_t start = block_excl_scan<kMaxBins>(len, sh[0], &tot_len);
  const uint64_t tb = block_excl_scan<kMaxBins>(nt, sh[1], &tot_nt);
  const uint64_t idx = block_excl_scan<kMaxBins>(used, sh[2], &tot_used);
  if (b < nb) btile[b] = (uint32_t)tb;
  if (used) {
    const int rb = (lut_rbits && lut_rbits[b] < rbits) ? lut_rbits[b] : rbits;
    big[idx] = Seg{(int64_t)start, (int64_t)len, rb, buf};
    nt_over[idx] = (int32_t)nt;
  }
  if (b == 0) ctr->n_big = tot_used;
}

__global__ __launch_bounds__(kMaxBins) void stripe_rows_kernel(const uint32_t* __restrict__ prun,
                                                               int nb,
                                                               uint32_t* __restrict__ rowtot) {
  __shared__ uint64_t sh[kMaxBins / 64 + 1];
  const int64_t s = blockIdx.x;
  const uint32_t b = threadIdx.x;
  const uint64_t my = b < (uint32_t)nb ? (prun[s * kMaxBins + b] + kTile - 1) / kTile : 0;
  uint64_t tot;
  block_excl_scan<kMaxBins>(my, sh, &tot);
  if (b == 0) rowtot[s] = (uint32_t)tot;
}

__global__ __launch_bounds__(kMaxBins) void stripe_order_kernel(
    const uint32_t* __restrict__ prun, const uint32_t* __restrict__ ptile,
    const uint32_t* __restrict__ btile, const uint32_t* __restrict__ rowtot, int nb,
    int32_t* __restrict__ torder) {
  __shared__ uint64_t sh[kMaxBins / 64 + 1];
  const int64_t s = blockIdx.x;
  const uint32_t b = threadIdx.x;
  uint64_t before = 0;
  for (int64_t i = b; i < s; i += kMaxBins) before += rowtot[i];
  uint64_t base;
  block_excl_scan<kMaxBins>(before, sh, &base);
  const uint32_t len = b < (uint32_t)nb ? prun[s * kMaxBins + b] : 0u;
  const uint64_t my = (len + kTile - 1) / kTile;
  uint64_t tot;
  uint64_t pos = base + block_excl_scan<kMaxBins>(my, sh, &tot);
  if (my) {
    const uint32_t t = btile[b] + ptile[s * kMaxBins + b];
    for (uint32_t c = 0; c < (uint32_t)my; c++) torder[pos + c] = (int32_t)(t + c);
  }
}

__global__ void stripe_gtile_kernel(const uint32_t* __restrict__ prun,
                                    const uint32_t* __restrict__ ptile,
                                    const uint32_t* __restrict__ btile,
                                    const uint64_t* __restrict__ sbase,
                                    const SegPlan* __restrict__ plan, int64_t nstripes, int nb,
                                    GTile* __restrict__ gt) {
  const int64_t i = (int64_t)blockIdx.x * blockDim.x + threadIdx.x;
  if (i >= nstripes * nb) return;
  const int64_t s = i / nb;
  const int b = (int)(i % nb);
  const uint32_t len = prun[s * kMaxBins + b];
  if (len == 0) return;
  const int64_t src = plan[s].start + (int64_t)sbase[s * kMaxBins + b];
  GTile* out = gt + btile[b] + ptile[s * kMaxBins + b];
  for (uint32_t c = 0; c * (uint32_t)kTile < len; c++) {
    const uint32_t rem = len - c * (uint32_t)kTile;
    out[c] = GTile{src + (int64_t)c * kTile, (int32_t)(rem < (uint32_t)kTile ? rem : kTile), 0};
  }
}

template <int LUT>
struct ScatterLds {
  uint64_t sval[kTile];
  uint16_t sdig[(LUT == 1 || !SRS_SCATTER_SDIG) ? 1 : kTile];
  alignas(8) uint16_t wc[kScatterThreads / 64][kMaxBins];
  uint16_t bin_start[kMaxBins];
  int64_t gdst[kMaxBins];
  uint32_t scan_sh[kScatterThreads / 64 + 1];
};

struct TileInfo {
  int64_t base;
  int32_t cnt;
  int32_t s;
  int64_t t;
};

#ifdef SRS_DIAG_LOOKBACK
__device__ __forceinline__ void diag_lookback(const SortDesc* __restrict__ desc,
                                              const SegPlan& P, int64_t t, uint32_t d,
                                              uint32_t tb, int64_t my_off,
                                              const uint64_t* __restrict__ offs,
                                              const uint32_t* __restrict__ offs32) {
  uint32_t* st = desc->lb_status;
  const uint64_t first = offs32 ? offs32[P.tile_base * kMaxBins + d] : offs[P.tile_base * kMaxBins + d];
  uint32_t pre = 0;
  if (t == P.tile_base) {
    __hip_atomic_store(&st[t * kMaxBins + d], (2u << 30) | tb, __ATOMIC_RELAXED,
                       __HIP_MEMORY_SCOPE_AGENT);
  } else {
    __hip_atomic_store(&st[t * kMaxBins + d], (1u << 30) | tb, __ATOMIC_RELAXED,
                       __HIP_MEMORY_SCOPE_AGENT);
    int64_t j = t - 1;
    uint32_t spins = 0, hops = 0;
    while (true) {
      const uint32_t v = __hip_atomic_load(&st[j * kMaxBins + d], __ATOMIC_RELAXED,
                                           __HIP_MEMORY_SCOPE_AGENT);
      const uint32_t f = v >> 30;
      if (f == 0) {
        if (++spins > (1u << 22)) {
          atomicAdd(&desc->lb_err[1], 1ull);
          break;
        }
        __builtin_amdgcn_s_sleep(1);
        continue;
      }
      pre += v & 0x3FFFFFFFu;
      hops++;
      if (f == 2 || j == P.tile_base) break;
      j--;
    }
    __hip_atomic_store(&st[t * kMaxBins + d], (2u << 30) | (pre + tb), __ATOMIC_RELAXED,
                       __HIP_MEMORY_SCOPE_AGENT);
    if (d == 0) atomicAdd(&desc->lb_err[2], (unsigned long long)hops);
  }
  if ((uint64_t)my_off - first != pre) atomicAdd(&desc->lb_err[0], 1ull);
}
#endif

template <typename KT, typename U, bool PRE3>
__device__ __forceinline__ TileInfo scatter_load_tile(
    const SortDesc* __restrict__ desc, const SegPlan* __restrict__ plan,
    const int32_t* __restrict__ tile_seg, const uint64_t* __restrict__ offs,
    const uint32_t* __restrict__ offs32, const GTile* __restrict__ gt, int64_t t, int ncols,
    uint64_t (&v0)[kScatterItems], uint64_t (&v1)[kScatterItems],
    uint64_t (&v2)[kScatterItems], int64_t& my_off) {
  constexpr int IT = kScatterItems;
  TileInfo ti;
  ti.t = t;
  ti.s = tile_seg[t];
  const SegPlan P = plan[ti.s];
  if (gt) {
    ti.base = gt[t].src;
    ti.cnt = gt[t].cnt;
  } else {
    const int64_t tl = t - P.tile_base;
    ti.base = P.start + tl * kTile;
    const int64_t rem = P.len - tl * kTile;
    ti.cnt = P.skip ? 0 : (rem < kTile ? (int)rem : kTile);
  }
  const int ebase = (int)(threadIdx.x >> 6) * IT * 64 + (int)lane_id();
  constexpr int LA = SRS_SCATTER_LOAD_AUX;
  load_strip<IT, false, 0, LA>(v0, desc->cols[0].base[P.buf], desc->cols[0].width,
                               desc->cols[0].stride[P.buf], ti.base, ebase, ti.cnt);
  const bool pair_src = PRE3 && desc->pair && (P.buf == BUF_TMP || P.buf == BUF_TMP2);
  if (ncols > 1)
    load_strip<IT, false, 0, LA>(v1, desc->cols[1].base[P.buf], pair_src ? 8u : desc->cols[1].width,
                                 desc->cols[1].stride[P.buf], ti.base, ebase, ti.cnt);
  if (PRE3 && ncols > 2 && !pair_src)
    load_strip<IT, false, 0, LA>(v2, desc->cols[2].base[P.buf], desc->cols[2].width,
                                 desc->cols[2].stride[P.buf], ti.base, ebase, ti.cnt);
  my_off = 0;
  if (ti.cnt > 0 && threadIdx.x < (1u << P.bits))
    my_off = offs32 ? (int64_t)offs32[t * kMaxBins + threadIdx.x]
                    : (int64_t)offs[t * kMaxBins + threadIdx.x];
  return ti;
}

template <typename KT, typename U, int LUT, bool CZ, bool PRE3>
__device__ __forceinline__ void scatter_process_tile(
    const SortDesc* __restrict__ desc, const SegPlan* __restrict__ plan, ScatterLds<LUT>& L,
    const TileInfo& ti, int ncols, const uint64_t (&v0)[kScatterItems],
    uint64_t (&v1)[kScatterItems], uint64_t (&v2)[kScatterItems], int64_t my_off,
    const DigitLut& lut, const uint64_t* __restrict__ lb_offs = nullptr,
    const uint32_t* __restrict__ lb_offs32 = nullptr) {
  constexpr int NT = kScatterThreads;
  constexpr int IT = kScatterItems;
  constexpr int NW = NT / 64;
  const SegPlan P = plan[ti.s];
  const uint32_t nb = 1u << P.bits;
  const uint32_t mask = nb - 1;
  const uint32_t wave = threadIdx.x >> 6;
  const int ebase = (int)wave * IT * 64 + (int)lane_id();
  const int cnt = ti.cnt;
  Xform<U, CZ> xf;
  xf.init(*desc);
  const int kbytes = desc->key_bits >> 3;
  const uint64_t kmask = kbytes == 8 ? ~0ull : ((1ull << (8 * kbytes)) - 1);
  STAMP_DECL
  STAMP();

  if constexpr (LUT) lds_barrier();
  static_assert(kMaxBins % 256 == 0, "row zeroing: 64 lanes x u64");
#pragma unroll
  for (int i = 0; i < kMaxBins / 256; i++)
    ((uint64_t*)&L.wc[wave][0])[i * 64 + lane_id()] = 0;
  auto valid = [&](int k) -> bool { return ebase + k * 64 < cnt; };
  uint32_t dg[IT];
#pragma unroll
  for (int k = 0; k < IT; k++) dg[k] = pass_digit<LUT>(xf((U)(v0[k] & kmask)), P.shift, mask, lut);
  STAMP();

  uint32_t pos[IT];
  wlms_rank_fn<IT, kMaxDigitBits, true>([&](int k) { return dg[k]; }, valid, P.bits,
                                        &L.wc[wave][0], pos);
  lds_barrier();
  STAMP();

  {
    const uint32_t my_bin = threadIdx.x;
    uint32_t tb = 0;
    if (my_bin < nb) {
#pragma unroll
      for (int w = 0; w < NW; w++) {
        const uint32_t c = L.wc[w][my_bin];
        L.wc[w][my_bin] = (uint16_t)tb;
        tb += c;
      }
    }
    const uint32_t ex = block_excl_scan_1b<NT>(tb, L.scan_sh);
    if (my_bin < nb) {
      L.bin_start[my_bin] = ex;
      L.gdst[my_bin] = P.start + my_off - (int64_t)ex;
    }
#ifdef SRS_DIAG_LOOKBACK
    if (my_bin < nb && desc->lb_status)
      diag_lookback(desc, P, ti.t, my_bin, tb, my_off, lb_offs, lb_offs32);
#endif
  }
  lds_barrier();
  STAMP();

#pragma unroll
  for (int k = 0; k < IT; k++) {
    if (valid(k)) {
      const uint32_t d = dg[k];
      pos[k] = L.bin_start[d] + L.wc[wave][d] + pos[k];
      L.sval[pos[k]] = v0[k];
      if constexpr (LUT != 1 && SRS_SCATTER_SDIG) L.sdig[pos[k]] = (uint16_t)d;
    }
  }
  lds_barrier();
  STAMP();

#ifdef SRS_DIAG_WIN
  auto diag_win = [&](int j, uint32_t d) -> int64_t {
    constexpr int S = SRS_DIAG_WIN;
    const int64_t tl = (ti.base - P.start) / kTile;
    const int64_t wb = P.start + (tl / S) * S * kTile;
    const int64_t per = (int64_t)S * kTile >> P.bits;
    const int64_t r = ((tl % S) * (per / S) + (j - (int)L.bin_start[d])) % per;
    const int64_t a = wb + (int64_t)d * per + r;
    return a < P.start + P.len ? a : ti.base + j;
  };
#endif
  uint16_t dout[IT];
  {
    char* out = desc->cols[0].base[P.dst];
    const uint32_t w = desc->cols[0].width, st = desc->cols[0].stride[P.dst];
    with_width(w, [&](auto W_) {
#pragma unroll
      for (int i = 0; i < IT; i++) {
        const int j = i * NT + (int)threadIdx.x;
        dout[i] = 0;
        if (j < cnt) {
          const uint64_t x = L.sval[j];
          uint32_t d;
          if constexpr (LUT == 1 || !SRS_SCATTER_SDIG) d = pass_digit<LUT>(xf((U)(x & kmask)), P.shift, mask, lut);
          else d = L.sdig[j];
          dout[i] = (uint16_t)d;
          #ifdef SRS_DIAG_SEQW
          stw<decltype(W_)::value>(out + ((int64_t)j + ti.base) * (int64_t)st, x);
#elif defined(SRS_DIAG_WIN)
          stw<decltype(W_)::value>(out + diag_win(j, d) * (int64_t)st, x);
#else
          stw<decltype(W_)::value>(out + ((int64_t)j + L.gdst[d]) * (int64_t)st, x);
#endif
        }
      }
    });
  }
  constexpr int STEP = PRE3 ? 2 : 1;
  auto move_col = [&](int c, uint64_t (&v)[IT]) {
    const uint32_t cw = desc->cols[c].width, cst = desc->cols[c].stride[P.dst];
    lds_barrier();
#pragma unroll
    for (int k = 0; k < IT; k++)
      if (valid(k)) L.sval[pos[k]] = v[k];
    lds_barrier();
    if (c + STEP < ncols)
      load_strip<IT, false, 0, SRS_SCATTER_LOAD_AUX>(
          v, desc->cols[c + STEP].base[P.buf], desc->cols[c + STEP].width,
          desc->cols[c + STEP].stride[P.buf], ti.base, ebase, cnt);
    char* out = desc->cols[c].base[P.dst];
    with_width(cw, [&](auto W_) {
#pragma unroll
      for (int i = 0; i < IT; i++) {
        const int j = i * NT + (int)threadIdx.x;
        if (j < cnt)
          #ifdef SRS_DIAG_SEQW
          stw<decltype(W_)::value>(out + ((int64_t)j + ti.base) * (int64_t)cst, L.sval[j]);
#elif defined(SRS_DIAG_WIN)
          stw<decltype(W_)::value>(out + diag_win(j, dout[i]) * (int64_t)cst, L.sval[j]);
#else
          stw<decltype(W_)::value>(out + ((int64_t)j + L.gdst[dout[i]]) * (int64_t)cst,
                                   L.sval[j]);
#endif
      }
    });
  };
  if constexpr (PRE3) {
    if (desc->pair) {
      if (P.buf != BUF_TMP && P.buf != BUF_TMP2) {
#pragma unroll
        for (int k = 0; k < IT; k++) v1[k] = (v1[k] & 0xFFFFFFFFull) | (v2[k] << 32);
      }
      lds_barrier();
#pragma unroll
      for (int k = 0; k < IT; k++)
        if (valid(k)) L.sval[pos[k]] = v1[k];
      lds_barrier();
      char* out = desc->cols[1].base[P.dst];
#pragma unroll
      for (int i = 0; i < IT; i++) {
        const int j = i * NT + (int)threadIdx.x;
        if (j < cnt) stw<8>(out + ((int64_t)j + L.gdst[dout[i]]) * 8, L.sval[j]);
      }
    } else {
      for (int c = 1; c < ncols; c += 2) {
        move_col(c, v1);
        if (c + 1 < ncols) move_col(c + 1, v2);
      }
    }
  } else {
    for (int c = 1; c < ncols; c++) move_col(c, v1);
  }
  STAMP();
  STAMP_FLUSH(0);
}

template <typename KT, typename U, int LUT, bool CZ, bool PRE3>
__global__ __launch_bounds__(kScatterThreads, SRS_SCATTER_WAVES_PER_EU) void scatter_kernel(
    const SortDesc* __restrict__ desc, const SegPlan* __restrict__ plan,
    const int32_t* __restrict__ tile_seg, const uint64_t* __restrict__ offs,
    const uint32_t* __restrict__ offs32, const GTile* __restrict__ gt) {
  __shared__ ScatterLds<LUT> L;
  __shared__ alignas(16) uint16_t slut[kLutLdsEntries<LUT>];
  const int64_t t = xcd_remap(blockIdx.x, gridDim.x);
  const int ncols = desc->ncols;
  uint64_t v0[kScatterItems], v1[kScatterItems], v2[kScatterItems];
  int64_t my_off;
  const TileInfo ti = scatter_load_tile<KT, U, PRE3>(desc, plan, tile_seg, offs, offs32, gt, t,
                                                     ncols, v0, v1, v2, my_off);
  if (ti.cnt == 0) return;
  const DigitLut lut = stage_lut<LUT, kScatterThreads>(desc, slut);
  scatter_process_tile<KT, U, LUT, CZ, PRE3>(desc, plan, L, ti, ncols, v0, v1, v2, my_off, lut,
                                             offs, offs32);
}

constexpr int kPairThreads = 512;
constexpr int kPairItems = 16;
constexpr int kPairTile = 2 * kTile;
static_assert(kPairThreads * kPairItems == kPairTile, "tile pair shape");
static_assert(kPairThreads >= kMaxBins, "the pair scan gives one bin per thread");

struct PairLds {
  uint64_t sval[kPairTile];
  alignas(8) uint16_t wc[kPairThreads / 64][kMaxBins];
  uint16_t bin_start[kMaxBins];
  int64_t gdst[kMaxBins];
  uint32_t scan_sh[kPairThreads / 64 + 1];
};

template <int IT, typename T>
__device__ __forceinline__ void load_strip_t(T (&dst)[IT], const char* src, uint32_t w,
                                             uint32_t st, int64_t first, int ebase, int cnt) {
  uint64_t tmp[IT];
  load_strip<IT>(tmp, src, w, st, first, ebase, cnt);
#pragma unroll
  for (int k = 0; k < IT; k++) dst[k] = (T)tmp[k];
}

template <typename KT, typename U, int LUT>
__device__ __forceinline__ void scatter_pair_tiles(
    const SortDesc* __restrict__ desc, const SegPlan* __restrict__ plan, PairLds& L,
    const int32_t* __restrict__ tile_seg, const uint64_t* __restrict__ offs,
    const uint32_t* __restrict__ offs32, const GTile* __restrict__ gt, int64_t ta, int64_t tb,
    const DigitLut& lut) {
  constexpr int NT = kPairThreads;
  constexpr int IT = kPairItems;
  constexpr int NW = NT / 64;
  constexpr int KW = sizeof(KT) >= 8 ? 8 : 4;
  typedef typename std::conditional<KW == 8, uint64_t, uint32_t>::type KR;
  const SegPlan P = plan[tile_seg[ta]];
  int64_t base[2] = {0, 0};
  int cnt[2] = {0, 0};
  for (int h = 0; h < 2; h++) {
    const int64_t t = h ? tb : ta;
    if (t < 0) continue;
    if (gt) {
      base[h] = gt[t].src;
      cnt[h] = gt[t].cnt;
    } else {
      const int64_t tl = t - P.tile_base;
      base[h] = P.start + tl * kTile;
      const int64_t rem = P.len - tl * kTile;
      cnt[h] = P.skip ? 0 : (int)std::min<int64_t>(rem, kTile);
    }
  }
  const int total = cnt[0] + cnt[1];
  if (total == 0) return;
  const uint32_t wave = threadIdx.x >> 6;
  const int half = (int)(wave >> 2);
  const int64_t mybase = half ? base[1] : base[0];
  const int mycnt = half ? cnt[1] : cnt[0];
  const int ebase = (int)(wave & 3) * IT * 64 + (int)lane_id();
  const int ncols = desc->ncols;
  const bool pair = desc->pair != 0;
  const bool pair_src = pair && (P.buf == BUF_TMP || P.buf == BUF_TMP2);

  KR v0[IT];
  uint64_t v1[IT];
  load_strip_t<IT>(v0, desc->cols[0].base[P.buf], desc->cols[0].width,
                   desc->cols[0].stride[P.buf], mybase, ebase, mycnt);
  if (ncols > 1)
    load_strip<IT>(v1, desc->cols[1].base[P.buf], pair_src ? 8u : desc->cols[1].width,
                   desc->cols[1].stride[P.buf], mybase, ebase, mycnt);
  if (pair && !pair_src) {
    uint32_t v2[IT];
    load_strip_t<IT>(v2, desc->cols[2].base[P.buf], 4u, desc->cols[2].stride[P.buf], mybase,
                     ebase, mycnt);
#pragma unroll
    for (int k = 0; k < IT; k++) v1[k] = (v1[k] & 0xFFFFFFFFull) | ((uint64_t)v2[k] << 32);
  }
  int64_t my_off = 0;
  const uint32_t nb = 1u << P.bits;
  if (threadIdx.x < nb)
    my_off = offs32 ? (int64_t)offs32[ta * kMaxBins + threadIdx.x]
                    : (int64_t)offs[ta * kMaxBins + threadIdx.x];

  const uint32_t mask = nb - 1;
  Xform<U, false> xf;
  xf.init(*desc);
  const int kbytes = desc->key_bits >> 3;
  const U kmask = kbytes >= (int)sizeof(U) ? (U)~(U)0 : (U)(((uint64_t)1 << (8 * kbytes)) - 1);
#pragma unroll
  for (int i = 0; i < kMaxBins / 256; i++)
    ((uint64_t*)&L.wc[wave][0])[i * 64 + lane_id()] = 0;
  auto valid = [&](int k) -> bool { return ebase + k * 64 < mycnt; };
  uint32_t dg[IT];
#pragma unroll
  for (int k = 0; k < IT; k++) dg[k] = pass_digit<LUT>(xf((U)v0[k] & kmask), P.shift, mask, lut);
  uint32_t pos[IT];
  wlms_rank_fn<IT, kMaxDigitBits, true>([&](int k) { return dg[k]; }, valid, P.bits,
                                        &L.wc[wave][0], pos);
  lds_barrier();
  {
    const uint32_t my_bin = threadIdx.x;
    uint32_t tsum = 0;
    if (my_bin < nb) {
#pragma unroll
      for (int w = 0; w < NW; w++) {
        const uint32_t c = L.wc[w][my_bin];
        L.wc[w][my_bin] = (uint16_t)tsum;
        tsum += c;
      }
    }
    const uint32_t ex = block_excl_scan_1b<NT>(tsum, L.scan_sh);
    if (my_bin < nb) {
      L.bin_start[my_bin] = (uint16_t)ex;
      L.gdst[my_bin] = P.start + my_off - (int64_t)ex;
    }
  }
  lds_barrier();
  KR* skey = (KR*)L.sval;
  uint16_t* sdig = (uint16_t*)((char*)L.sval + (size_t)kPairTile * 4);
#pragma unroll
  for (int k = 0; k < IT; k++)
    if (valid(k)) {
      const uint32_t d = dg[k];
      pos[k] = L.bin_start[d] + L.wc[wave][d] + pos[k];
      skey[pos[k]] = v0[k];
      if constexpr (KW == 4) sdig[pos[k]] = (uint16_t)d;
    }
  lds_barrier();
  uint16_t dout[IT];
  {
    char* out = desc->cols[0].base[P.dst];
    const uint32_t st = desc->cols[0].stride[P.dst];
    with_width(desc->cols[0].width, [&](auto W_) {
#pragma unroll
      for (int i = 0; i < IT; i++) {
        const int j = i * NT + (int)threadIdx.x;
        dout[i] = 0;
        if (j < total) {
          const KR x = skey[j];
          uint32_t d;
          if constexpr (KW == 4) d = sdig[j];
          else d = pass_digit<LUT>(xf((U)x & kmask), P.shift, mask, lut);
          dout[i] = (uint16_t)d;
          stw<decltype(W_)::value>(out + ((int64_t)j + L.gdst[d]) * (int64_t)st, (uint64_t)x);
        }
      }
    });
  }
  if (ncols < 2) return;
  lds_barrier();
#pragma unroll
  for (int k = 0; k < IT; k++)
    if (valid(k)) L.sval[pos[k]] = v1[k];
  lds_barrier();
  {
    char* out = desc->cols[1].base[P.dst];
    const bool pair_dst = pair && (P.dst == BUF_TMP || P.dst == BUF_TMP2);
// ... 2112 lines not shown
}

__global__ __launch_bounds__(kMaxBins) void super_apply_kernel(const SegPlan* __restrict__ plan,
                                                               const uint32_t* __restrict__ gsum,
                                                               int64_t ngroups,
                                                               const uint64_t* __restrict__ sofs,
                                                               uint64_t* __restrict__ gofs) {
  const uint32_t b = threadIdx.x;
  if (plan[0].skip || b >= (1u << plan[0].bits)) return;
  const int64_t g0 = (int64_t)blockIdx.x * kSuperGroups;
  const int64_t g1 = min(g0 + kSuperGroups, ngroups);
  uint64_t run = sofs[(int64_t)blockIdx.x * kMaxBins + b];
  for (int64_t g = g0; g < g1; g++) {
    gofs[g * kMaxBins + b] = run;
    run += gsum[g * kMaxBins + b];
  }
}

void launch_offsets(SegPlan* plan, int64_t nbig, const int32_t* group_seg, int64_t ngroups,
                    const uint16_t* hist, uint32_t* gsum, uint64_t* gofs, uint64_t* sbase,
                    uint64_t* offs, uint32_t* offs32, const unsigned long long* var_or,
                    Seg* big_next,
                    Seg* local, Seg* local2, Seg* copy, ListCounters* ctr,
                    const int32_t* lut_rbits, hipStream_t st, int mode, uint32_t* prun) {
  group_sum_kernel<<<(unsigned)ngroups, kMaxBins, 0, st>>>(plan, group_seg, hist, gsum);
  if (nbig == 1 && mode != 1 && ngroups >= g_super_min_groups && super_scan_enabled()) {
    const int64_t ns = super_rows(ngroups);
    uint32_t* ssum = gsum + ngroups * kMaxBins;
    uint64_t* sofs = gofs + ngroups * kMaxBins;
    super_sum_kernel<<<(unsigned)ns, kMaxBins, 0, st>>>(plan, gsum, ngroups, ssum);
    seg_scan_kernel<<<1, kMaxBins, 0, st>>>(plan, ssum, sofs, sbase, var_or, big_next, local,
                                            local2, copy, ctr, lut_rbits, mode, prun, ns);
    super_apply_kernel<<<(unsigned)ns, kMaxBins, 0, st>>>(plan, gsum, ngroups, sofs, gofs);
  } else {
    seg_scan_kernel<<<(unsigned)nbig, kMaxBins, 0, st>>>(plan, gsum, gofs, sbase, var_or,
                                                        big_next, local, local2, copy, ctr,
                                                        lut_rbits, mode, prun, 0);
  }
  tile_offs_kernel<<<(unsigned)ngroups, kMaxBins, 0, st>>>(
      plan, group_seg, hist, gofs, sbase, offs, offs32);
}

void launch_scatter(int key_size, const SortDesc* d, const SegPlan* plan,
                    const int32_t* tile_seg, const uint64_t* offs, const uint32_t* offs32,
                    int64_t ntiles, int lut, int ncols, hipStream_t st, const GTile* gt) {
  const bool pre3 = ncols >= 3;
#define CALL_L(KT, U, CZ, LK)                                                           \
  if (pre3)                                                                             \
    scatter_kernel<KT, U, LK, CZ, true><<<(unsigned)ntiles, kScatterThreads, 0, st>>>(    \
        d, plan, tile_seg, offs, offs32, gt);                                           \
  else                                                                                  \
    scatter_kernel<KT, U, LK, CZ, false><<<(unsigned)ntiles, kScatterThreads, 0, st>>>(   \
        d, plan, tile_seg, offs, offs32, gt)
#define CALL(KT, U, CZ)                                                                 \
  if (lut == 2) {                                                                       \
    CALL_L(KT, U, CZ, 2);                                                               \
  } else if (lut) {                                                                     \
    CALL_L(KT, U, CZ, 1);                                                               \
  } else {                                                                              \
    CALL_L(KT, U, CZ, 0);                                                               \
  }
  SRS_KEY_DISPATCH(key_size, CALL)
#undef CALL
#undef CALL_L
}

void launch_scatter_pairs(int key_size, const SortDesc* d, const SegPlan* plan,
                          const int32_t* tile_seg, const uint64_t* offs, const uint32_t* offs32,
                          int64_t ntiles, int lut, hipStream_t st, const GTile* gt) {
  const unsigned grid = (unsigned)((ntiles + 1) / 2);
#define CALL_P(KT, U, LK)                                                            \
  scatter_pair_kernel<KT, U, LK><<<grid, kPairThreads, 0, st>>>(d, plan, tile_seg, offs, \
                                                               offs32, gt, ntiles)
  if (key_size == 4) {
    if (lut == 2) CALL_P(uint32_t, uint32_t, 2);
    else CALL_P(uint32_t, uint32_t, 0);
  } else {
    if (lut == 2) CALL_P(uint64_t, uint64_t, 2);
    else CALL_P(uint64_t, uint64_t, 0);
  }
#undef CALL_P
}

void launch_stripe_tables(const uint32_t* prun, int64_t nstripes, int nb, uint32_t* ptile,
                          uint64_t* btot, uint32_t* bnt, int rbits, int buf, Seg* big,
                          int32_t* nt_over, uint32_t* btile, ListCounters* ctr,
                          const uint64_t* sbase, const SegPlan* plan, GTile* gt,
                          const int32_t* lut_rbits, hipStream_t st, int32_t* torder,
                          int64_t tiles_cap) {
  stripe_tiles_kernel<<<(unsigned)nb, kStripeThreads, 0, st>>>(prun, nstripes, ptile, btot, bnt);
  stripe_segs_kernel<<<1, kMaxBins, 0, st>>>(btot, bnt, nb, rbits, buf, big, nt_over, btile, ctr,
                                             lut_rbits);
  const int64_t np = nstripes * nb;
  stripe_gtile_kernel<<<(unsigned)((np + 255) / 256), 256, 0, st>>>(prun, ptile, btile, sbase,
                                                                    plan, nstripes, nb, gt);
  if (torder) {
    uint32_t* rowtot = (uint32_t*)(torder + tiles_cap);
    stripe_rows_kernel<<<(unsigned)nstripes, kMaxBins, 0, st>>>(prun, nb, rowtot);
    stripe_order_kernel<<<(unsigned)nstripes, kMaxBins, 0, st>>>(prun, ptile, btile, rowtot, nb,
                                                                 torder);
  }
}

void launch_local(int key_size, const SortDesc* d, const Seg* segs, int64_t nsegs, int big_class,
                  Seg* fallback, unsigned long long* fallback_count, hipStream_t st,
                  bool rec16) {
#define CALL_R(KT, U, CZ, R)                                                                \
  if (big_class)                                                                            \
    local_kernel<KT, U, kLocalThreads, kLocalItems, kLocalWavesPerEU, CZ, R>                \
        <<<(unsigned)nsegs, kLocalThreads, 0, st>>>(d, segs, fallback, fallback_count);     \
  else                                                                                      \
    local_kernel<KT, U, kLocalThreadsSmall, kLocalItemsSmall, kLocalWavesPerEUSmall, CZ, R> \
        <<<(unsigned)nsegs, kLocalThreadsSmall, 0, st>>>(d, segs, fallback, fallback_count)
#define CALL(KT, U, CZ) \
  if (rec16) { CALL_R(KT, U, CZ, true); } else { CALL_R(KT, U, CZ, false); }
  SRS_KEY_DISPATCH(key_size, CALL)
#undef CALL
#undef CALL_R
}

void launch_local_direct(int key_size, int pm, const SortDesc* d, const Seg* segs,
                         int64_t nsegs, Seg* redo, unsigned long long* redo_count, Seg* fallback,
                         unsigned long long* fallback_count, hipStream_t st, bool big) {
#define CALL(KT, PM)                                                                          \
  if (big)                                                                                    \
    local_direct_kernel<KT, KT, kLocalDirectThreads2, kLocalDirectItems2,                     \
                        kLocalDirectWavesPerEU2, PM>                                          \
        <<<(unsigned)nsegs, kLocalDirectThreads2, 0, st>>>(d, segs, redo, redo_count,         \
                                                           fallback, fallback_count, xcd);    \
  else                                                                                        \
    local_direct_kernel<KT, KT, kLocalDirectThreads, kLocalDirectItems,                       \
                        kLocalDirectWavesPerEU, PM>                                           \
        <<<(unsigned)nsegs, kLocalDirectThreads, 0, st>>>(d, segs, redo, redo_count,          \
                                                          fallback, fallback_count, xcd)
  static const int xcd = [] {
    const char* e = getenv("SRS_LOCAL_XCD");
    return (e && *e == '0') ? 0 : 1;
  }();
  if (pm == 1) {
    CALL(uint64_t, 1);
  } else if (pm == 2) {
    CALL(uint32_t, 2);
  } else if (key_size == 4) {
    CALL(uint32_t, 0);
  } else {
    CALL(uint64_t, 0);
  }
#undef CALL
}

void launch_local_list(int key_size, const SortDesc* d, const Seg* segs,
                       const unsigned long long* nsegs, int grid, Seg* fallback,
                       unsigned long long* fallback_count, hipStream_t st, bool big) {
  if (big && key_size == 4)
    local_list_kernel<uint32_t, uint32_t, kLocalThreads, kLocalItems, kLocalWavesPerEU>
        <<<(unsigned)grid, kLocalThreads, 0, st>>>(d, segs, nsegs, fallback, fallback_count);
  else if (big)
    local_list_kernel<uint64_t, uint64_t, kLocalThreads, kLocalItems, kLocalWavesPerEU>
        <<<(unsigned)grid, kLocalThreads, 0, st>>>(d, segs, nsegs, fallback, fallback_count);
  else if (key_size == 4)
    local_list_kernel<uint32_t, uint32_t, kLocalThreadsSmall, kLocalItemsSmall,
                      kLocalWavesPerEUSmall>
        <<<(unsigned)grid, kLocalThreadsSmall, 0, st>>>(d, segs, nsegs, fallback, fallback_count);
  else
    local_list_kernel<uint64_t, uint64_t, kLocalThreadsSmall, kLocalItemsSmall,
                      kLocalWavesPerEUSmall>
        <<<(unsigned)grid, kLocalThreadsSmall, 0, st>>>(d, segs, nsegs, fallback, fallback_count);
}

void launch_local_stable(int key_size, const SortDesc* d, const Seg* segs,
                         const unsigned long long* nsegs, int big_class, Seg* fallback,
                         unsigned long long* fallback_count, int grid, hipStream_t st) {
#define CALL(KT, U, CZ)                                                                \
  if (big_class)                                                                       \
    local_stable_kernel<KT, U, kLocalStableThreads, CZ>                                \
        <<<(unsigned)grid, kLocalStableThreads, 0, st>>>(d, segs, nsegs, fallback,      \
                                                         fallback_count);              \
  else                                                                                 \
    local_stable_kernel<KT, U, kLocalStableThreadsSmall, CZ>                           \
        <<<(unsigned)grid, kLocalStableThreadsSmall, 0, st>>>(d, segs, nsegs, fallback, \
                                                             fallback_count)
  SRS_KEY_DISPATCH(key_size, CALL)
#undef CALL
// ... 875 lines not shown
```

### simd-radix-sort_amd/python/srs_amd/__init__.py

```python
from __future__ import annotations

import ctypes
import os

import numpy as np

try:
    import torch
    _HAVE_TORCH = True
except Exception:
    _HAVE_TORCH = False

_PKG_ROOT = os.path.dirname(os.path.dirname(os.path.dirname(os.path.abspath(__file__))))
LIB_PATH = os.environ.get("SRS_AMD_LIB") or os.path.join(_PKG_ROOT, "lib", "libsrs_amd.so")

KEY_U8, KEY_I8, KEY_U16, KEY_I16, KEY_U32, KEY_I32, KEY_U64, KEY_I64, KEY_F32, KEY_F64 = range(10)
_NP_KIND = {np.dtype(np.uint8): KEY_U8, np.dtype(np.int8): KEY_I8,
            np.dtype(np.uint16): KEY_U16, np.dtype(np.int16): KEY_I16,
            np.dtype(np.uint32): KEY_U32, np.dtype(np.int32): KEY_I32,
            np.dtype(np.uint64): KEY_U64, np.dtype(np.int64): KEY_I64,
            np.dtype(np.float32): KEY_F32, np.dtype(np.float64): KEY_F64}

SRS_OK = 0
LEAF_SORTED, LEAF_UNSORTED = 0, 1
_LEAF = {"insertion": LEAF_SORTED, "bramas": LEAF_SORTED, "nosort": LEAF_UNSORTED}


class SrsError(RuntimeError):
    pass


_lib = None


def lib() -> ctypes.CDLL:
    global _lib
    if _lib is not None:
        return _lib
    if not os.path.exists(LIB_PATH):
        raise ImportError(f"libsrs_amd.so not built: {LIB_PATH} (run `make -C simd-radix-sort_amd`)")
    L = ctypes.CDLL(LIB_PATH)
    i64, i32, u32, vp = ctypes.c_int64, ctypes.c_int32, ctypes.c_uint32, ctypes.c_void_p
    L.srs_sort_soa.argtypes = [i64, ctypes.c_int, ctypes.c_int, i64, vp, i32, vp, vp]
    L.srs_sort_aos.argtypes = [i64, ctypes.c_int, ctypes.c_int, i64, vp, u32]
    L.srs_sort_soa_leaf.argtypes = [i64, ctypes.c_int, ctypes.c_int, i64, ctypes.c_int, vp, i32,
                                    vp, vp]
    L.srs_sort_aos_leaf.argtypes = [i64, ctypes.c_int, ctypes.c_int, i64, ctypes.c_int, vp, u32]
    L.srs_sort_soa_device_leaf.argtypes = [i64, ctypes.c_int, ctypes.c_int, i64, ctypes.c_int, vp,
                                           i32, vp, vp, vp, vp, vp]
    L.srs_sort_aos_device_leaf.argtypes = [i64, ctypes.c_int, ctypes.c_int, i64, ctypes.c_int, vp,
                                           u32, vp, vp]
    L.srs_sort_soa_device.argtypes = [i64, ctypes.c_int, ctypes.c_int, i64, vp, i32, vp, vp,
                                      vp, vp, vp]
    L.srs_sort_aos_device.argtypes = [i64, ctypes.c_int, ctypes.c_int, i64, vp, u32, vp, vp]
    L.srs_sort_segments_device.argtypes = [i64, ctypes.c_int, ctypes.c_int, vp, i32, vp, vp, i64,
                                           vp, i32, vp]
    L.srs_topk_soa_device.argtypes = [i64, i64, ctypes.c_int, ctypes.c_int, vp, i32, vp, vp, vp,
                                      vp, vp, vp]
    L.srs_topk_aos_device.argtypes = [i64, i64, ctypes.c_int, ctypes.c_int, vp, u32, vp, vp, vp]
    L.srs_debug_set_topk_candidates.argtypes = [i64]
    L.srs_debug_last_topk.argtypes = [ctypes.POINTER(i64)]
    L.srs_topk_rows_soa_device.argtypes = [i64, i64, i64, i64, ctypes.c_int, ctypes.c_int, vp, i32,
                                           vp, vp, vp, vp, vp, vp]
    L.srs_topk_rows_max_k.restype = i64
    L.srs_debug_set_topk_rows_route.argtypes = [ctypes.c_int]
    L.srs_debug_last_topk_rows.argtypes = [ctypes.POINTER(i64)]
    L.srs_fill_synthetic_device.argtypes = [i64, ctypes.c_int, ctypes.c_uint64, ctypes.c_uint64,
                                            vp, i32, vp, vp, vp]
    L.srs_key_histogram_device.argtypes = [i64, ctypes.c_int, ctypes.c_int, vp, ctypes.c_int, vp,
                                           vp]
    L.srs_partition_device.argtypes = [i64, ctypes.c_int, ctypes.c_int, vp, i32, vp, vp,
                                       ctypes.c_int, vp, i32, vp, vp, vp, vp]
    L.srs_debug_last_fallbacks.argtypes = [ctypes.POINTER(i64)]
    L.srs_debug_set_super_scan.argtypes = [i64]
    L.srs_debug_last_local_counts.argtypes = [ctypes.POINTER(i64)]
    L.srs_debug_last_local_classes.argtypes = [ctypes.POINTER(i64)]
    L.srs_set_host_devices.argtypes = [i32, vp]
    L.srs_last_error.restype = ctypes.c_char_p
    L.srs_version.restype = ctypes.c_char_p
    L.srs_set_kernel_timing.argtypes = [ctypes.c_int]
    L.srs_kernel_stats.argtypes = [ctypes.c_char_p, ctypes.POINTER(i64),
                                   ctypes.POINTER(ctypes.c_double),
                                   ctypes.POINTER(ctypes.c_double)]
    L.srs_debug_alloc.argtypes = [ctypes.c_uint64, ctypes.c_int, ctypes.POINTER(vp)]
    L.srs_debug_free.argtypes = [vp]
    L.srs_alloc_device.argtypes = [ctypes.c_uint64, ctypes.POINTER(vp)]
    L.srs_free_device.argtypes = [vp]
    L.srs_debug_probe_write.argtypes = [vp, ctypes.c_uint64, ctypes.POINTER(ctypes.c_float)]
    L.srs_debug_workspace.argtypes = [ctypes.POINTER(vp), ctypes.POINTER(ctypes.c_uint64),
                                      ctypes.POINTER(vp), ctypes.POINTER(ctypes.c_uint64)]
    _lib = L
    return L


def _check(rc: int):
    if rc != SRS_OK:
        raise SrsError(f"srs error {rc}: {lib().srs_last_error().decode()}")


def version() -> str:
    return lib().srs_version().decode()


def key_kind_of(dtype) -> int:
    dt = np.dtype(dtype)
    if dt not in _NP_KIND:
        raise TypeError(f"unsupported key dtype {dt}")
    return _NP_KIND[dt]


def _ptr_array(ptrs):
    return (ctypes.c_void_p * max(1, len(ptrs)))(*ptrs)


def _size_array(sizes):
    return (ctypes.c_uint32 * max(1, len(sizes)))(*sizes)


def _leaf(cmp_sorter: str) -> int:
    if cmp_sorter not in _LEAF:
        raise ValueError(f"cmp_sorter must be one of {sorted(_LEAF)}")
    return _LEAF[cmp_sorter]


def sort_thresh(cmp_sort_threshold: int, keys: np.ndarray, *payloads: np.ndarray,
                up: bool = True, cmp_sorter: str = "insertion") -> None:
    n = len(keys)
    for a in (keys,) + payloads:
        if not (isinstance(a, np.ndarray) and a.flags.c_contiguous and a.ndim == 1):
            raise ValueError("arrays must be 1-D C-contiguous numpy arrays")
        if len(a) != n:
            raise ValueError("all arrays must have the same length")
    _check(lib().srs_sort_soa_leaf(n, key_kind_of(keys.dtype), int(bool(up)),
                                   int(cmp_sort_threshold), _leaf(cmp_sorter), keys.ctypes.data,
                                   len(payloads), _ptr_array([p.ctypes.data for p in payloads]),
                                   _size_array([p.dtype.itemsize for p in payloads])))


def set_host_devices(devices=()) -> None:
    d = [int(x) for x in devices]
    arr = (ctypes.c_int32 * max(1, len(d)))(*d)
    _check(lib().srs_set_host_devices(len(d), arr))


def sort(keys: np.ndarray, *payloads: np.ndarray, up: bool = True) -> None:
    sort_thresh(16, keys, *payloads, up=up)


def sort_combined(elements: np.ndarray, key_kind: int, up: bool = True,
                  cmp_sort_threshold: int = 16, cmp_sorter: str = "insertion") -> None:
    if not elements.flags.c_contiguous:
        raise ValueError("elements must be C-contiguous")
    n = elements.shape[0]
    esz = elements.nbytes // n if n else elements.dtype.itemsize
    _check(lib().srs_sort_aos_leaf(n, int(key_kind), int(bool(up)), int(cmp_sort_threshold),
                                   _leaf(cmp_sorter), elements.ctypes.data, esz))


_TORCH_KIND = None
# ... 198 lines not shown
                                               keys.data_ptr(), len(payloads),
                                               _ptr_array([p.data_ptr() for p in payloads]),
                                               _size_array([p.element_size() for p in payloads]),
                                               _stream_ptr(stream, keys.device)))


def key_histogram_device(keys, hist, bits: int, up: bool = True, key_kind: int | None = None,
                         stream=None) -> None:
    kind = _torch_kind(keys) if key_kind is None else int(key_kind)
    if hist.numel() != (1 << bits) or hist.element_size() != 8 or not hist.is_cuda:
        raise ValueError("hist must be a device tensor of 2^bits 64-bit counters")
    _check_columns(keys, (keys,))
    if hist.device != keys.device or not hist.is_contiguous():
        raise ValueError("hist must be contiguous and on the keys' GPU")
    with _on_device(keys):
        _check(lib().srs_key_histogram_device(keys.numel(), kind, int(bool(up)), keys.data_ptr(),
                                              int(bits), hist.data_ptr(),
                                              _stream_ptr(stream, keys.device)))


def partition_device(keys, payloads, bits: int, part_of_bucket, num_parts: int, out,
                     up: bool = True, key_kind: int | None = None, stream=None):
    kind = _torch_kind(keys) if key_kind is None else int(key_kind)
    if part_of_bucket.dtype.itemsize != 4 or part_of_bucket.numel() != (1 << bits):
        raise ValueError("part_of_bucket must hold 2^bits int32 entries")
    pays = list(payloads)
    _check_columns(keys, [keys] + pays)
    if not (part_of_bucket.is_cuda and part_of_bucket.device == keys.device and
            part_of_bucket.is_contiguous()):
        raise ValueError("part_of_bucket must be a contiguous tensor on the keys' GPU")
    if len(out) != 1 + len(pays):
        raise ValueError("out must hold keys_out followed by every payload_out")
    for o, i in zip(out, [keys] + pays):
        if not (o.is_cuda and o.device == keys.device and o.is_contiguous() and o.dim() == 1 and
                o.numel() >= keys.numel() and o.element_size() == i.element_size()):
            raise ValueError("out tensors must be contiguous, on the keys' GPU, at least as long "
                             "as the input and of its element size")
    counts = (ctypes.c_int64 * num_parts)()
    with _on_device(keys):
        _check(lib().srs_partition_device(
            keys.numel(), kind, int(bool(up)), keys.data_ptr(), len(pays),
            _ptr_array([p.data_ptr() for p in pays]), _size_array([p.element_size() for p in pays]),
            int(bits), part_of_bucket.data_ptr(), int(num_parts), out[0].data_ptr(),
            _ptr_array([o.data_ptr() for o in out[1:]]), counts,
            _stream_ptr(stream, keys.device)))
    return [int(c) for c in counts]


def set_kernel_timing(enable) -> None:
    _check(lib().srs_set_kernel_timing(2 if enable == 2 else int(bool(enable))))


def reset_kernel_stats() -> None:
    _check(lib().srs_reset_kernel_stats())


def kernel_stats(name: str):
    n = ctypes.c_int64()
    ms = ctypes.c_double()
    el = ctypes.c_double()
    _check(lib().srs_kernel_stats(name.encode(), ctypes.byref(n), ctypes.byref(ms),
                                  ctypes.byref(el)))
    return n.value, ms.value, el.value


def last_fallbacks():
    c = (ctypes.c_int64 * 2)()
    _check(lib().srs_debug_last_fallbacks(c))
    return int(c[0]), int(c[1])


def last_local_counts():
    c = (ctypes.c_int64 * 2)()
    _check(lib().srs_debug_last_local_counts(c))
    return int(c[0]), int(c[1])


def last_local_classes():
    c = (ctypes.c_int64 * 4)()
    _check(lib().srs_debug_last_local_classes(c))
    return tuple(int(x) for x in c)


class _DeviceBlock:

    def __init__(self, n, dtype, device):
        import torch
        self.device = torch.device(device)
        self.dtype = dtype
        self.n = int(n)
        nbytes = self.n * torch.empty(0, dtype=dtype).element_size()
        p = ctypes.c_void_p()
        with torch.cuda.device(self.device):
            _check(lib().srs_alloc_device(nbytes, ctypes.byref(p)))
        self.ptr = int(p.value or 0)
        typestr = {torch.int64: "<i8", torch.int32: "<i4", torch.float32: "<f4",
                   torch.float64: "<f8", torch.int16: "<i2", torch.uint8: "|u1",
                   torch.int8: "|i1"}[dtype]
        self.__cuda_array_interface__ = {"shape": (self.n,), "typestr": typestr,
                                         "data": (self.ptr, False), "version": 2,
                                         "strides": None}

    def __del__(self):
        if getattr(self, "ptr", 0):
            try:
                lib().srs_free_device(ctypes.c_void_p(self.ptr))
            except Exception:
                pass
            self.ptr = 0


def empty_device(n: int, dtype, device="cuda"):
    import torch
    blk = _DeviceBlock(n, dtype, device)
    t = torch.as_tensor(blk, device=blk.device)
    if t.data_ptr() != blk.ptr:
        raise SrsError("empty_device: torch copied the block instead of viewing it")
    t._srs_block = blk
    return t


def debug_alloc(nbytes: int, mode: int = 0) -> int:
    p = ctypes.c_void_p()
    _check(lib().srs_debug_alloc(int(nbytes), int(mode), ctypes.byref(p)))
    return int(p.value)


def debug_free(ptr: int) -> None:
    _check(lib().srs_debug_free(ctypes.c_void_p(ptr)))


def debug_set_super_scan(min_groups: int) -> None:
    _check(lib().srs_debug_set_super_scan(int(min_groups)))


def debug_set_topk_candidates(max_candidates: int) -> None:
    _check(lib().srs_debug_set_topk_candidates(int(max_candidates)))


def debug_last_topk():
    c = (ctypes.c_int64 * 3)()
    _check(lib().srs_debug_last_topk(c))
    return int(c[0]), int(c[1]), int(c[2])


def debug_set_topk_rows_route(route: int) -> None:
    _check(lib().srs_debug_set_topk_rows_route(int(route)))


def debug_last_topk_rows():
    c = (ctypes.c_int64 * 4)()
    _check(lib().srs_debug_last_topk_rows(c))
    return tuple(int(x) for x in c)


def debug_probe_write(ptr: int, nbytes: int) -> float:
    ms = ctypes.c_float()
    _check(lib().srs_debug_probe_write(ctypes.c_void_p(ptr), int(nbytes), ctypes.byref(ms)))
    return float(ms.value)


def debug_workspace():
    a, b = ctypes.c_void_p(), ctypes.c_void_p()
    na, nb = ctypes.c_uint64(), ctypes.c_uint64()
    _check(lib().srs_debug_workspace(ctypes.byref(a), ctypes.byref(na), ctypes.byref(b),
                                     ctypes.byref(nb)))
# ... 6 lines not shown
```

Baseline: 48.74 Gkeys/s.

## Pack partial stripe tails into two-range gather tiles to cut tile count

Adds a stripe packing pass that merges the leftover tail of one stripe's bucket run with the head of the next stripe's run into a single gather tile. A tile can now describe two source ranges (GTile gains src1/cnt1), and the loaders in the count, scatter and merge kernels remap element offsets past cnt0 by a delta. This is meant to cut the number of partially filled tiles and the per-tile overhead in the striped first level. In exchange, the tile-table build runs its packing scan on a single thread per bucket, and the loads pay extra offset arithmetic. A debug API for counting tiles is also added.

```diff
diff --git a/include/srs_c_api.h b/include/srs_c_api.h
--- a/include/srs_c_api.h
+++ b/include/srs_c_api.h
@@ -168,6 +168,8 @@
 
 int srs_debug_last_local_classes(int64_t* counts);
 
+int srs_debug_last_gather_tiles(int64_t* counts);
+
 int srs_debug_alloc(uint64_t bytes, int mode, void** ptr);
 int srs_debug_free(void* ptr);
 int srs_debug_workspace(void** tmp, uint64_t* tmp_bytes, void** tmp2, uint64_t* tmp2_bytes);
diff --git a/simd-radix-sort_amd/csrc/srs_api.hip b/simd-radix-sort_amd/csrc/srs_api.hip
--- a/simd-radix-sort_amd/csrc/srs_api.hip
+++ b/simd-radix-sort_amd/csrc/srs_api.hip
@@ -464,6 +464,7 @@
   DevBuf shist, lut, lut_rbits;
   DevBuf prun, ptile, btot, bnt, btile, nt_over, gtile, gorder;
   int64_t gorder_cap = 0;
+  int gather_nb = 0;
   DevBuf mid;
   DevBuf midbar;
   DevBuf sel, selhist, selcnt, seldesc;
@@ -1077,6 +1078,8 @@
   const GTile* gt = nullptr;
   const int32_t* nt_over = nullptr;
   const int32_t* torder = nullptr;
+  int pack = 1;
+  int64_t span_max = 0;
   int key_bits = 0;
   bool home = false;
 };
@@ -1190,7 +1193,8 @@
                          (uint64_t*)W->btot.p, (uint32_t*)W->bnt.p, rbits, BUF_TMP,
                          (Seg*)W->big[nxt].p, (int32_t*)W->nt_over.p, (uint32_t*)W->btile.p,
                          d_ctr, (const uint64_t*)W->sbase.p, plan, (GTile*)W->gtile.p,
-                         lut_rbits, st, (int32_t*)W->gorder.p, W->gorder_cap);
+                         lut_rbits, st, (int32_t*)W->gorder.p, W->gorder_cap, M.pack, M.span_max);
+    W->gather_nb = nb;
   }
   HIP_TRY(hipMemcpyAsync(W->h_ctr, d_ctr, sizeof(ListCounters), hipMemcpyDeviceToHost, st));
   SRS_TRY(sync_poll(st));
@@ -1347,6 +1351,11 @@
 
 constexpr int64_t kStripeMinN = int64_t(1) << 25;
 
+bool gather_pack_enabled() {
+  const char* e = getenv("SRS_GATHER_PACK");
+  return !(e && *e == '0');
+}
+
 bool stripes_enabled() {
   static const bool on = [] {
     const char* e = getenv("SRS_NO_STRIPES");
@@ -1498,6 +1507,7 @@
     set_xcd_rotation(e && *e ? atoi(e) : 0);
   }
   W->last_small = false;
+  W->gather_nb = 0;
   const int ks = key_size_of(R.kind);
   const int64_t n = R.num;
   const bool inplace = is_inplace(R);
@@ -1750,9 +1760,9 @@
     const int nb = 1 << b1;
     const size_t pieces = (size_t)K * kMaxBins;
     SRS_TRY(ensure(W->prun, pieces * 4));
-    SRS_TRY(ensure(W->ptile, pieces * 4));
+    SRS_TRY(ensure(W->ptile, pieces * 16));
     SRS_TRY(ensure(W->btot, kMaxBins * 8));
-    SRS_TRY(ensure(W->bnt, kMaxBins * 4));
+    SRS_TRY(ensure(W->bnt, 2 * kMaxBins * 4));
     SRS_TRY(ensure(W->btile, kMaxBins * 4));
     SRS_TRY(ensure(W->nt_over, kMaxBins * 4));
     SRS_TRY(ensure(W->gtile, ((n + kTile - 1) / kTile + (size_t)K * nb) * sizeof(GTile)));
@@ -1764,6 +1774,12 @@
     LevelMode m1;
     m1.mode = 1;
     m1.key_bits = d.key_bits;
+    m1.pack = gather_pack_enabled();
+    {
+      uint32_t stride = std::max(d.key.stride[BUF_TMP], d.pair ? 8u : 0u);
+      for (int c = 0; c < d.ncols; c++) stride = std::max(stride, d.cols[c].stride[BUF_TMP]);
+      m1.span_max = (int64_t)0x7FFFFFFF / std::max(stride, 1u);
+    }
     ++level;
     if (balanced)
       SRS_TRY(run_level(W, ksl, d_desc, S, kMaxDigitBits, d.lut_mode >= 2 ? 2 : 1, st,
@@ -3238,6 +3254,23 @@
   return SRS_OK;
 }
 
+int srs_debug_last_gather_tiles(int64_t* counts) {
+  if (!counts) return fail(SRS_ERR_INVALID_ARG, "counts is NULL");
+  Workspace* W = nullptr;
+  WsLock lk;
+  SRS_TRY(acquire_ws(&W, &lk));
+  counts[0] = counts[1] = 0;
+  if (W->last_small || W->gather_nb == 0 || !W->bnt.p) return SRS_OK;
+  HIP_TRY(hipDeviceSynchronize());
+  std::vector<uint32_t> h(2 * kMaxBins);
+  HIP_TRY(hipMemcpy(h.data(), W->bnt.p, h.size() * 4, hipMemcpyDeviceToHost));
+  for (int b = 0; b < W->gather_nb; b++) {
+    counts[0] += h[b];
+    counts[1] += h[kMaxBins + b];
+  }
+  return SRS_OK;
+}
+
 int srs_debug_set_super_scan(int64_t min_groups) {
   set_super_scan_min_groups(min_groups);
   return SRS_OK;
diff --git a/simd-radix-sort_amd/csrc/srs_common.h b/simd-radix-sort_amd/csrc/srs_common.h
--- a/simd-radix-sort_amd/csrc/srs_common.h
+++ b/simd-radix-sort_amd/csrc/srs_common.h
@@ -60,9 +60,10 @@
 };
 
 struct GTile {
-  int64_t src;
-  int32_t cnt;
-  int32_t pad;
+  int64_t src0;
+  int64_t src1;
+  int32_t cnt0;
+  int32_t cnt1;
 };
 #ifndef SRS_STRIPE_KPB
 #define SRS_STRIPE_KPB 3904
diff --git a/simd-radix-sort_amd/csrc/srs_kernels.h b/simd-radix-sort_amd/csrc/srs_kernels.h
--- a/simd-radix-sort_amd/csrc/srs_kernels.h
+++ b/simd-radix-sort_amd/csrc/srs_kernels.h
@@ -44,12 +44,13 @@
 void launch_scatter_pairs(int key_size, const SortDesc* d, const SegPlan* plan,
                           const int32_t* tile_seg, const uint64_t* offs, const uint32_t* offs32,
                           int64_t ntiles, int lut, hipStream_t st, const GTile* gt = nullptr);
-void launch_stripe_tables(const uint32_t* prun, int64_t nstripes, int nb, uint32_t* ptile,
+void launch_stripe_tables(const uint32_t* prun, int64_t nstripes, int nb, uint32_t* pp,
                           uint64_t* btot, uint32_t* bnt, int rbits, int buf, Seg* big,
                           int32_t* nt_over, uint32_t* btile, ListCounters* ctr,
                           const uint64_t* sbase, const SegPlan* plan, GTile* gt,
-                          const int32_t* lut_rbits, hipStream_t st, int32_t* torder = nullptr,
-                          int64_t tiles_cap = 0);
+                          const int32_t* lut_rbits, hipStream_t st, int32_t* torder,
+                          int64_t tiles_cap,
+                          int pack, int64_t span_max);
 void launch_key_hist(int key_size, int64_t n, const void* keys, const SortDesc& d, int bits,
                      unsigned long long* hist, hipStream_t st);
 void launch_local(int key_size, const SortDesc* d, const Seg* segs, int64_t nsegs, int big_class,
diff --git a/simd-radix-sort_amd/csrc/srs_kernels.hip b/simd-radix-sort_amd/csrc/srs_kernels.hip
--- a/simd-radix-sort_amd/csrc/srs_kernels.hip
+++ b/simd-radix-sort_amd/csrc/srs_kernels.hip
@@ -118,6 +118,33 @@
     for (int k = 0; k < IT; k++) {
       if constexpr (D) dst[k] = bld<W, AUX>(r, o0 + (uint32_t)k * 64u * W);
       else dst[k] = bld<W, AUX>(r, o0, __builtin_amdgcn_readfirstlane((uint32_t)k * 64u * st));
+    }
+  });
+}
+
+template <int IT, bool BRANCH, bool DENSE = false, int FW = 0, int AUX = 0>
+__device__ __forceinline__ void load_strip_g(uint64_t (&dst)[IT], const char* src, uint32_t w,
+                                             uint32_t st, int64_t first, int ebase, int cnt,
+                                             int cnt0, int delta) {
+  if constexpr (BRANCH) {
+    if (cnt0 == cnt) {
+      load_strip<IT, DENSE, FW, AUX>(dst, src, w, st, first, ebase, cnt);
+      return;
+    }
+  }
+  const __amdgpu_buffer_rsrc_t r =
+      strip_rsrc(src + first * (int64_t)st, cnt > 0 ? (uint32_t)(cnt + delta) * st : 0u);
+  with_strip<IT, DENSE, FW>(w, st, [&](auto W_, auto D_) {
+    constexpr int W = decltype(W_)::value;
+    constexpr bool D = decltype(D_)::value;
+    const uint32_t es = D ? (uint32_t)W : st;
+    const uint32_t oa = (uint32_t)ebase * es, db = (uint32_t)delta * es;
+#pragma unroll
+    for (int k = 0; k < IT; k++) {
+      const uint32_t o = oa + (ebase + k * 64 >= cnt0 ? db : 0u);
+      if constexpr (D) dst[k] = bld<W, AUX>(r, o + (uint32_t)k * 64u * W);
+      else dst[k] = bld<W, AUX>(r, o, __builtin_amdgcn_readfirstlane((uint32_t)k * 64u * st));
+      if constexpr (!BRANCH) __builtin_amdgcn_sched_barrier(0);
     }
   });
 }
@@ -632,6 +659,7 @@
   int64_t t;
   int32_t s;
   int32_t cnt;
+  int32_t cnt0;
   bool vec;
 };
 
@@ -652,6 +680,7 @@
   CountTile T;
   T.t = t;
   T.cnt = 0;
+  T.cnt0 = 0;
   T.s = 0;
   T.vec = false;
   if (t >= ntiles) {
@@ -664,29 +693,37 @@
   const char* kp = desc->key.base[P.buf];
   const uint32_t ks = desc->key.stride[P.buf];
   int64_t base;
+  int delta = 0;
   if (gt) {
-    base = gt[t].src;
-    T.cnt = gt[t].cnt;
+    const GTile g = gt[t];
+    base = g.src0;
+    T.cnt = g.cnt0 + g.cnt1;
+    T.cnt0 = g.cnt0;
+    if (g.cnt1) delta = (int)(g.src1 - g.src0 - g.cnt0);
   } else {
     const int64_t tl = t - P.tile_base;
     base = P.start + tl * kTile;
     const int64_t rem = P.len - tl * kTile;
     T.cnt = rem < kTile ? (int)rem : kTile;
+    T.cnt0 = T.cnt;
   }
   constexpr int KB = (int)sizeof(KT);
   constexpr int PER = KB >= 4 ? 16 / KB : 1;
   static_assert(kCountItems % PER == 0, "whole 16-byte pieces per thread");
+  static_assert(PER <= 4, "GTile: a two-range tile's cnt0 is a multiple of 4");
   T.vec = KB >= 4 && ks == (uint32_t)KB;
   const int cnt = T.cnt;
   if (T.vec) {
     typedef uint32_t u32x4 __attribute__((ext_vector_type(4)));
+    u32x4 c[kCountItems / PER];
     const __amdgpu_buffer_rsrc_t r =
-        strip_rsrc(kp + base * (int64_t)KB, cnt > 0 ? (uint32_t)cnt * KB : 0u);
-    u32x4 c[kCountItems / PER];
+        strip_rsrc(kp + base * (int64_t)KB, cnt > 0 ? (uint32_t)(cnt + delta) * KB : 0u);
+    const uint32_t oa = threadIdx.x * 16u, ob = oa + (uint32_t)delta * KB;
+    const int thr = T.cnt0 * KB - (int)oa;
 #pragma unroll
     for (int j = 0; j < kCountItems / PER; j++)
       c[j] = __builtin_amdgcn_raw_buffer_load_b128(
-          r, (threadIdx.x + (uint32_t)j * kCountThreads) * 16u, 0, 0);
+          r, (j * kCountThreads * 16 >= thr ? ob : oa) + (uint32_t)j * kCountThreads * 16u, 0, 0);
 #pragma unroll
     for (int k = 0; k < kCountItems; k++) {
       const u32x4 v = c[k / PER];
@@ -699,7 +736,8 @@
 #pragma unroll
     for (int k = 0; k < kCountItems; k++) {
       const int e = count_elem<KT>(false, k);
-      raw[k] = e < cnt ? (U)gld<KT>(kp + (base + e) * (int64_t)ks) : (U)0;
+      raw[k] = e < cnt ? (U)gld<KT>(kp + (base + e + (e >= T.cnt0 ? delta : 0)) * (int64_t)ks)
+                       : (U)0;
     }
   }
   return T;
@@ -1083,27 +1121,85 @@
 }
 
 constexpr int kStripeThreads = 256;
-__global__ __launch_bounds__(kStripeThreads) void stripe_tiles_kernel(
-    const uint32_t* __restrict__ prun, int64_t nstripes, uint32_t* __restrict__ ptile,
-    uint64_t* __restrict__ btot, uint32_t* __restrict__ bnt) {
-  __shared__ uint64_t sh[kStripeThreads / 64 + 1];
-  __shared__ uint64_t sh2[kStripeThreads / 64 + 1];
+constexpr int kPackChunk = 1024;
+__global__ __launch_bounds__(kStripeThreads) void stripe_pack_kernel(
+    const uint32_t* __restrict__ prun, const uint64_t* __restrict__ sbase,
+    const SegPlan* __restrict__ plan, int64_t nstripes, int pack, int64_t span_max,
+    uint32_t* __restrict__ pp, uint64_t* __restrict__ btot, uint32_t* __restrict__ bnt) {
+  __shared__ int64_t ssrc[kPackChunk];
+  __shared__ uint32_t slen[kPackChunk], sfirst[kPackChunk], snt[kPackChunk], shc[kPackChunk],
+      snext[kPackChunk];
   const int b = blockIdx.x;
-  uint64_t tiles = 0, keys = 0;
-  for (int64_t s0 = 0; s0 < nstripes; s0 += kStripeThreads) {
-    const int64_t s = s0 + threadIdx.x;
-    const uint32_t len = s < nstripes ? prun[s * kMaxBins + b] : 0u;
-    const uint64_t nt = (len + kTile - 1) / kTile;
-    uint64_t tt, kt;
-    const uint64_t ex = block_excl_scan<kStripeThreads>(nt, sh, &tt);
-    block_excl_scan<kStripeThreads>((uint64_t)len, sh2, &kt);
-    if (s < nstripes) ptile[s * kMaxBins + b] = (uint32_t)(tiles + ex);
-    tiles += tt;
-    keys += kt;
+  const int64_t np = nstripes * kMaxBins;
+  uint64_t keys = 0;
+  uint32_t tiles = 0, two = 0;
+  for (int64_t s0 = 0; s0 < nstripes; s0 += kPackChunk) {
+    const int m = (int)min((int64_t)kPackChunk, nstripes - s0);
+    for (int i = threadIdx.x; i < m; i += kStripeThreads) {
+      const int64_t s = s0 + i;
+      slen[i] = prun[s * kMaxBins + b];
+      ssrc[i] = plan[s].start + (int64_t)sbase[s * kMaxBins + b];
+    }
+    __syncthreads();
+    if (threadIdx.x == 0) {
+      int open = -1;
+      uint32_t ocnt = 0;
+      int64_t oend = 0;
+      uint32_t len = slen[0];
+      int64_t src = ssrc[0];
+      for (int i = 0; i < m; i++) {
+        const uint32_t l = len;
+        const int64_t p = src;
+        if (i + 1 < m) {
+          len = slen[i + 1];
+          src = ssrc[i + 1];
+        }
+        uint32_t head = 0;
+        if (open >= 0 && l > 0) {
+          uint32_t take = 0;
+          if (p == oend || ocnt % 4 == 0) {
+            const uint32_t room = (uint32_t)kTile - ocnt;
+            take = l < room ? l : room;
+            const uint32_t adj = take < l ? (4 - (l - take) % 4) % 4 : 0;
+            take = take > adj ? take - adj : 0;
+          }
+          if (take > 0 && p + take - (oend - ocnt) <= span_max) {
+            head = take;
+            shc[open] |= take << 16;
+            snext[open] = (uint32_t)(s0 + i);
+            two += p != oend;
+          }
+          open = -1;
+        }
+        const uint32_t rem = l - head;
+        const uint32_t nt = (rem + kTile - 1) / kTile;
+        sfirst[i] = tiles;
+        snt[i] = nt;
+        shc[i] = head;
+        snext[i] = 0;
+        tiles += nt;
+        keys += l;
+        if (pack && rem % kTile) {
+          open = i;
+          ocnt = rem % kTile;
+          oend = p + l;
+        }
+      }
+    }
+    __syncthreads();
+    for (int i = threadIdx.x; i < m; i += kStripeThreads) {
+      const int64_t q = (s0 + i) * kMaxBins + b;
+      pp[q] = sfirst[i];
+      pp[np + q] = snt[i];
+      pp[2 * np + q] = shc[i];
+      pp[3 * np + q] = snext[i];
+    }
+    __syncthreads();
   }
   if (threadIdx.x == 0) {
     btot[b] = keys;
-    bnt[b] = (uint32_t)tiles;
+    bnt[b] = tiles;
+    bnt[kMaxBins + b] = two;
   }
 }
 
@@ -1130,20 +1226,20 @@
   if (b == 0) ctr->n_big = tot_used;
 }
 
-__global__ __launch_bounds__(kMaxBins) void stripe_rows_kernel(const uint32_t* __restrict__ prun,
+__global__ __launch_bounds__(kMaxBins) void stripe_rows_kernel(const uint32_t* __restrict__ pnt,
                                                                int nb,
                                                                uint32_t* __restrict__ rowtot) {
   __shared__ uint64_t sh[kMaxBins / 64 + 1];
   const int64_t s = blockIdx.x;
   const uint32_t b = threadIdx.x;
-  const uint64_t my = b < (uint32_t)nb ? (prun[s * kMaxBins + b] + kTile - 1) / kTile : 0;
+  const uint64_t my = b < (uint32_t)nb ? pnt[s * kMaxBins + b] : 0;
   uint64_t tot;
   block_excl_scan<kMaxBins>(my, sh, &tot);
   if (b == 0) rowtot[s] = (uint32_t)tot;
 }
 
 __global__ __launch_bounds__(kMaxBins) void stripe_order_kernel(
-    const uint32_t* __restrict__ prun, const uint32_t* __restrict__ ptile,
+    const uint32_t* __restrict__ pnt, const uint32_t* __restrict__ ptile,
     const uint32_t* __restrict__ btile, const uint32_t* __restrict__ rowtot, int nb,
     int32_t* __restrict__ torder) {
   __shared__ uint64_t sh[kMaxBins / 64 + 1];
@@ -1153,8 +1249,7 @@
   for (int64_t i = b; i < s; i += kMaxBins) before += rowtot[i];
   uint64_t base;
   block_excl_scan<kMaxBins>(before, sh, &base);
-  const uint32_t len = b < (uint32_t)nb ? prun[s * kMaxBins + b] : 0u;
-  const uint64_t my = (len + kTile - 1) / kTile;
+  const uint64_t my = b < (uint32_t)nb ? pnt[s * kMaxBins + b] : 0u;
   uint64_t tot;
   uint64_t pos = base + block_excl_scan<kMaxBins>(my, sh, &tot);
   if (my) {
@@ -1164,7 +1259,7 @@
 }
 
 __global__ void stripe_gtile_kernel(const uint32_t* __restrict__ prun,
-                                    const uint32_t* __restrict__ ptile,
+                                    const uint32_t* __restrict__ pp,
                                     const uint32_t* __restrict__ btile,
                                     const uint64_t* __restrict__ sbase,
                                     const SegPlan* __restrict__ plan, int64_t nstripes, int nb,
@@ -1173,13 +1268,28 @@
   if (i >= nstripes * nb) return;
   const int64_t s = i / nb;
   const int b = (int)(i % nb);
-  const uint32_t len = prun[s * kMaxBins + b];
-  if (len == 0) return;
-  const int64_t src = plan[s].start + (int64_t)sbase[s * kMaxBins + b];
-  GTile* out = gt + btile[b] + ptile[s * kMaxBins + b];
-  for (uint32_t c = 0; c * (uint32_t)kTile < len; c++) {
+  const int64_t np = nstripes * kMaxBins, q = s * kMaxBins + b;
+  const uint32_t nt = pp[np + q];
+  if (nt == 0) return;
+  const uint32_t hc = pp[2 * np + q];
+  const uint32_t head = hc & 0xFFFFu, cnt1 = hc >> 16;
+  const uint32_t len = prun[q] - head;
+  const int64_t src = plan[s].start + (int64_t)sbase[q] + head;
+  GTile* out = gt + btile[b] + pp[q];
+  for (uint32_t c = 0; c < nt; c++) {
     const uint32_t rem = len - c * (uint32_t)kTile;
-    out[c] = GTile{src + (int64_t)c * kTile, (int32_t)(rem < (uint32_t)kTile ? rem : kTile), 0};
+    GTile g{src + (int64_t)c * kTile, 0, (int32_t)(rem < (uint32_t)kTile ? rem : kTile), 0};
+    if (c + 1 == nt && cnt1) {
+      const int64_t s1 = pp[3 * np + q];
+      const int64_t src1 = plan[s1].start + (int64_t)sbase[s1 * kMaxBins + b];
+      if (src1 == g.src0 + g.cnt0) {
+        g.cnt0 += (int32_t)cnt1;
+      } else {
+        g.src1 = src1;
+        g.cnt1 = (int32_t)cnt1;
+      }
+    }
+    out[c] = g;
   }
 }
 
@@ -1198,6 +1308,8 @@
   int32_t cnt;
   int32_t s;
   int64_t t;
+  int32_t cnt0;
+  int32_t delta;
 };
 
 #ifdef SRS_DIAG_LOOKBACK
@@ -1254,26 +1366,35 @@
   ti.t = t;
   ti.s = tile_seg[t];
   const SegPlan P = plan[ti.s];
+  ti.delta = 0;
   if (gt) {
-    ti.base = gt[t].src;
-    ti.cnt = gt[t].cnt;
+    const GTile g = gt[t];
+    ti.base = g.src0;
+    ti.cnt = g.cnt0 + g.cnt1;
+    ti.cnt0 = g.cnt0;
+    if (g.cnt1) ti.delta = (int)(g.src1 - g.src0 - g.cnt0);
   } else {
     const int64_t tl = t - P.tile_base;
     ti.base = P.start + tl * kTile;
     const int64_t rem = P.len - tl * kTile;
     ti.cnt = P.skip ? 0 : (rem < kTile ? (int)rem : kTile);
+    ti.cnt0 = ti.cnt;
   }
   const int ebase = (int)(threadIdx.x >> 6) * IT * 64 + (int)lane_id();
   constexpr int LA = SRS_SCATTER_LOAD_AUX;
-  load_strip<IT, false, 0, LA>(v0, desc->cols[0].base[P.buf], desc->cols[0].width,
-                               desc->cols[0].stride[P.buf], ti.base, ebase, ti.cnt);
+  load_strip_g<IT, false, false, 0, LA>(v0, desc->cols[0].base[P.buf], desc->cols[0].width,
+                                 desc->cols[0].stride[P.buf], ti.base, ebase, ti.cnt, ti.cnt0,
+                                 ti.delta);
   const bool pair_src = PRE3 && desc->pair && (P.buf == BUF_TMP || P.buf == BUF_TMP2);
   if (ncols > 1)
-    load_strip<IT, false, 0, LA>(v1, desc->cols[1].base[P.buf], pair_src ? 8u : desc->cols[1].width,
-                                 desc->cols[1].stride[P.buf], ti.base, ebase, ti.cnt);
+    load_strip_g<IT, false, false, 0, LA>(v1, desc->cols[1].base[P.buf],
+                                   pair_src ? 8u : desc->cols[1].width,
+                                   desc->cols[1].stride[P.buf], ti.base, ebase, ti.cnt, ti.cnt0,
+                                   ti.delta);
   if (PRE3 && ncols > 2 && !pair_src)
-    load_strip<IT, false, 0, LA>(v2, desc->cols[2].base[P.buf], desc->cols[2].width,
-                                 desc->cols[2].stride[P.buf], ti.base, ebase, ti.cnt);
+    load_strip_g<IT, false, false, 0, LA>(v2, desc->cols[2].base[P.buf], desc->cols[2].width,
+                                   desc->cols[2].stride[P.buf], ti.base, ebase, ti.cnt, ti.cnt0,
+                                   ti.delta);
   my_off = 0;
   if (ti.cnt > 0 && threadIdx.x < (1u << P.bits))
     my_off = offs32 ? (int64_t)offs32[t * kMaxBins + threadIdx.x]
@@ -1403,9 +1524,9 @@
       if (valid(k)) L.sval[pos[k]] = v[k];
     lds_barrier();
     if (c + STEP < ncols)
-      load_strip<IT, false, 0, SRS_SCATTER_LOAD_AUX>(
+      load_strip_g<IT, false, false, 0, SRS_SCATTER_LOAD_AUX>(
           v, desc->cols[c + STEP].base[P.buf], desc->cols[c + STEP].width,
-          desc->cols[c + STEP].stride[P.buf], ti.base, ebase, cnt);
+          desc->cols[c + STEP].stride[P.buf], ti.base, ebase, cnt, ti.cnt0, ti.delta);
     char* out = desc->cols[c].base[P.dst];
     with_width(cw, [&](auto W_) {
 #pragma unroll
@@ -1488,9 +1609,10 @@
 
 template <int IT, typename T>
 __device__ __forceinline__ void load_strip_t(T (&dst)[IT], const char* src, uint32_t w,
-                                             uint32_t st, int64_t first, int ebase, int cnt) {
+                                             uint32_t st, int64_t first, int ebase, int cnt,
+                                             int cnt0, int delta) {
   uint64_t tmp[IT];
-  load_strip<IT>(tmp, src, w, st, first, ebase, cnt);
+  load_strip_g<IT, true>(tmp, src, w, st, first, ebase, cnt, cnt0, delta);
 #pragma unroll
   for (int k = 0; k < IT; k++) dst[k] = (T)tmp[k];
 }
@@ -1509,17 +1631,22 @@
   const SegPlan P = plan[tile_seg[ta]];
   int64_t base[2] = {0, 0};
   int cnt[2] = {0, 0};
+  int cnt0[2] = {0, 0}, delta[2] = {0, 0};
   for (int h = 0; h < 2; h++) {
     const int64_t t = h ? tb : ta;
     if (t < 0) continue;
     if (gt) {
-      base[h] = gt[t].src;
-      cnt[h] = gt[t].cnt;
+      const GTile g = gt[t];
+      base[h] = g.src0;
+      cnt[h] = g.cnt0 + g.cnt1;
+      cnt0[h] = g.cnt0;
+      if (g.cnt1) delta[h] = (int)(g.src1 - g.src0 - g.cnt0);
     } else {
       const int64_t tl = t - P.tile_base;
       base[h] = P.start + tl * kTile;
       const int64_t rem = P.len - tl * kTile;
       cnt[h] = P.skip ? 0 : (int)std::min<int64_t>(rem, kTile);
+      cnt0[h] = cnt[h];
     }
   }
   const int total = cnt[0] + cnt[1];
@@ -1528,6 +1655,8 @@
   const int half = (int)(wave >> 2);
   const int64_t mybase = half ? base[1] : base[0];
   const int mycnt = half ? cnt[1] : cnt[0];
+  const int mycnt0 = half ? cnt0[1] : cnt0[0];
+  const int mydelta = half ? delta[1] : delta[0];
   const int ebase = (int)(wave & 3) * IT * 64 + (int)lane_id();
   const int ncols = desc->ncols;
   const bool pair = desc->pair != 0;
@@ -1536,14 +1665,14 @@
   KR v0[IT];
   uint64_t v1[IT];
   load_strip_t<IT>(v0, desc->cols[0].base[P.buf], desc->cols[0].width,
-                   desc->cols[0].stride[P.buf], mybase, ebase, mycnt);
+                   desc->cols[0].stride[P.buf], mybase, ebase, mycnt, mycnt0, mydelta);
   if (ncols > 1)
-    load_strip<IT>(v1, desc->cols[1].base[P.buf], pair_src ? 8u : desc->cols[1].width,
-                   desc->cols[1].stride[P.buf], mybase, ebase, mycnt);
+    load_strip_g<IT, true>(v1, desc->cols[1].base[P.buf], pair_src ? 8u : desc->cols[1].width,
+                     desc->cols[1].stride[P.buf], mybase, ebase, mycnt, mycnt0, mydelta);
   if (pair && !pair_src) {
     uint32_t v2[IT];
     load_strip_t<IT>(v2, desc->cols[2].base[P.buf], 4u, desc->cols[2].stride[P.buf], mybase,
-                     ebase, mycnt);
+                     ebase, mycnt, mycnt0, mydelta);
 #pragma unroll
     for (int k = 0; k < IT; k++) v1[k] = (v1[k] & 0xFFFFFFFFull) | ((uint64_t)v2[k] << 32);
   }
@@ -3822,23 +3951,25 @@
 #undef CALL_P
 }
 
-void launch_stripe_tables(const uint32_t* prun, int64_t nstripes, int nb, uint32_t* ptile,
+void launch_stripe_tables(const uint32_t* prun, int64_t nstripes, int nb, uint32_t* pp,
                           uint64_t* btot, uint32_t* bnt, int rbits, int buf, Seg* big,
                           int32_t* nt_over, uint32_t* btile, ListCounters* ctr,
                           const uint64_t* sbase, const SegPlan* plan, GTile* gt,
                           const int32_t* lut_rbits, hipStream_t st, int32_t* torder,
-                          int64_t tiles_cap) {
-  stripe_tiles_kernel<<<(unsigned)nb, kStripeThreads, 0, st>>>(prun, nstripes, ptile, btot, bnt);
+                          int64_t tiles_cap, int pack, int64_t span_max) {
+  const int64_t npieces = nstripes * kMaxBins;
+  stripe_pack_kernel<<<(unsigned)nb, kStripeThreads, 0, st>>>(prun, sbase, plan, nstripes, pack,
+                                                              span_max, pp, btot, bnt);
   stripe_segs_kernel<<<1, kMaxBins, 0, st>>>(btot, bnt, nb, rbits, buf, big, nt_over, btile, ctr,
                                              lut_rbits);
   const int64_t np = nstripes * nb;
-  stripe_gtile_kernel<<<(unsigned)((np + 255) / 256), 256, 0, st>>>(prun, ptile, btile, sbase,
-                                                                    plan, nstripes, nb, gt);
+  stripe_gtile_kernel<<<(unsigned)((np + 255) / 256), 256, 0, st>>>(prun, pp, btile, sbase, plan,
+                                                                    nstripes, nb, gt);
   if (torder) {
     uint32_t* rowtot = (uint32_t*)(torder + tiles_cap);
-    stripe_rows_kernel<<<(unsigned)nstripes, kMaxBins, 0, st>>>(prun, nb, rowtot);
-    stripe_order_kernel<<<(unsigned)nstripes, kMaxBins, 0, st>>>(prun, ptile, btile, rowtot, nb,
-                                                                 torder);
+    stripe_rows_kernel<<<(unsigned)nstripes, kMaxBins, 0, st>>>(pp + npieces, nb, rowtot);
+    stripe_order_kernel<<<(unsigned)nstripes, kMaxBins, 0, st>>>(pp + npieces, pp, btile, rowtot,
+                                                                 nb, torder);
   }
 }
 
diff --git a/simd-radix-sort_amd/python/srs_amd/__init__.py b/simd-radix-sort_amd/python/srs_amd/__init__.py
--- a/simd-radix-sort_amd/python/srs_amd/__init__.py
+++ b/simd-radix-sort_amd/python/srs_amd/__init__.py
@@ -75,6 +75,7 @@
     L.srs_debug_set_super_scan.argtypes = [i64]
     L.srs_debug_last_local_counts.argtypes = [ctypes.POINTER(i64)]
     L.srs_debug_last_local_classes.argtypes = [ctypes.POINTER(i64)]
+    L.srs_debug_last_gather_tiles.argtypes = [ctypes.POINTER(i64)]
     L.srs_set_host_devices.argtypes = [i32, vp]
     L.srs_last_error.restype = ctypes.c_char_p
     L.srs_version.restype = ctypes.c_char_p
@@ -439,6 +440,12 @@
     return tuple(int(x) for x in c)
 
 
+def last_gather_tiles():
+    c = (ctypes.c_int64 * 2)()
+    _check(lib().srs_debug_last_gather_tiles(c))
+    return int(c[0]), int(c[1])
+
+
 class _DeviceBlock:
 
     def __init__(self, n, dtype, device):
```

Result: no change. 48.30 Gkeys/s (-0.9%).
